# LIS-TU-Berlin/SVN-ICP

Hardware: AMD Instinct MI355X
Metric: scan-pair registrations/sec at N particles x M source pts, 1/2/4/8 GPU (higher is better)
Workload: dtype f64; 1 GPU; C3: 128 particles SVN-ICP, 131072-pt source vs 262144-pt target, K=100, I=20, max_dist=1.0, lr=1.0, SVNFullGrad=False, correspondence=fast, early stop off; synthetic 64-beam scans (seed 20250718); particles=128, target_points=262144, knn_count=100, parallelism=single GPU

## Files before the change

include/svnicp_hip.h:

```cpp
#ifndef SVNICP_HIP_H
#define SVNICP_HIP_H

#include <stdint.h>

#ifdef __cplusplus
extern "C" {
#endif

#define SVNICP_ABI_VERSION 1

typedef struct svnicp_ctx svnicp_ctx;

#define SVNICP_ALIGN_SUCCESS 1
#define SVNICP_NO_OPTIMIZER 2

typedef enum {
  SVNICP_OK = 0,
  SVNICP_ERR_INVALID = -1,
  SVNICP_ERR_HIP = -2,
  SVNICP_ERR_NO_DEVICE = -3,
  SVNICP_ERR_NOMEM = -4
} svnicp_status;

#define SVNICP_MODE_SVN 0
#define SVNICP_MODE_SVGD 1

#define SVNICP_OPT_ADAM 0
#define SVNICP_OPT_RMSPROP 1
#define SVNICP_OPT_SGD 2
#define SVNICP_OPT_ADAGRAD 3
#define SVNICP_OPT_NONE (-1)

#define SVNICP_MEM_HOST 0
#define SVNICP_MEM_DEVICE 1

typedef struct svnicp_params {
  int32_t struct_size;
  int32_t mode;
  int32_t iterations;
  int32_t knn_count;
  double lr;
  double max_dist;
  double convergence_threshold;
  int32_t check_early_stop;
  int32_t svn_full_grad;
  int32_t optimizer;
  int32_t record_trace;
} svnicp_params;

int svnicp_create(const svnicp_params *params, int device, const double *init_pose6xP, int P,
                  svnicp_ctx **out);
void svnicp_destroy(svnicp_ctx *ctx);
const char *svnicp_last_error(const svnicp_ctx *ctx);
int svnicp_abi_version(void);

#define SVNICP_OWN_STREAM ((void *)(intptr_t)-1)
int svnicp_set_stream(svnicp_ctx *ctx, void *hip_stream);
int svnicp_synchronize(svnicp_ctx *ctx);

int svnicp_set_clouds(svnicp_ctx *ctx, const double *src_xyz, int64_t B, const double *tgt_xyz,
                      int64_t M, int mem_kind);
int svnicp_set_particles(svnicp_ctx *ctx, const double *init_pose6xP, int P);
int svnicp_set_source(svnicp_ctx *ctx, const double *src_xyz, int64_t B, int mem_kind);
int svnicp_set_target(svnicp_ctx *ctx, const double *tgt_xyz, int64_t M, int mem_kind);

int svnicp_set_initial_mean(svnicp_ctx *ctx, const double R0_rowmajor[9], const double t0[3]);
int svnicp_set_k(svnicp_ctx *ctx, int k);
int svnicp_set_max_dist(svnicp_ctx *ctx, double max_dist);

int svnicp_align(svnicp_ctx *ctx);
int svnicp_align_async(svnicp_ctx *ctx);

int svnicp_get_transformation(svnicp_ctx *ctx, double out6[6]);
int svnicp_get_distribution(svnicp_ctx *ctx, double out6[6]);
int svnicp_get_cov_matrix(svnicp_ctx *ctx, double out36[36]);
int svnicp_get_particles(svnicp_ctx *ctx, double *out6P);
int svnicp_get_particle_weight(svnicp_ctx *ctx, double *outP);
int svnicp_get_particle_history(svnicp_ctx *ctx, float *outIx6P);
int svnicp_get_runtime(svnicp_ctx *ctx, double out3[3]);

int svnicp_set_option(svnicp_ctx *ctx, const char *name, const char *value);

int svnicp_set_shard(svnicp_ctx *ctx, int p_lo, int p_hi);
int svnicp_set_row_shard(svnicp_ctx *ctx, int row_rank, int row_world, int64_t total_source_points);
void *svnicp_rank_sums_devptr(svnicp_ctx *ctx);
int svnicp_align_begin(svnicp_ctx *ctx);
int svnicp_stage_candidates(svnicp_ctx *ctx, int64_t b_lo, int64_t b_hi);
int svnicp_build_candidate_table(svnicp_ctx *ctx);
int svnicp_iter_accumulate(svnicp_ctx *ctx, int iteration);
int svnicp_iter_update(svnicp_ctx *ctx, int iteration);
int svnicp_finish(svnicp_ctx *ctx);
int svnicp_stopped(svnicp_ctx *ctx);
void *svnicp_candidates_devptr(svnicp_ctx *ctx);
void *svnicp_sums_devptr(svnicp_ctx *ctx);
#define SVNICP_NSUMS 22

typedef struct svnicp_map svnicp_map;
int svnicp_map_create(int device, double voxel_size, double max_range, int max_points, int64_t capacity_voxels,
                      svnicp_map **out);
void svnicp_map_destroy(svnicp_map *map);
const char *svnicp_map_last_error(const svnicp_map *map);
int svnicp_map_clear(svnicp_map *map);
int svnicp_map_size(svnicp_map *map, int64_t *voxels);
int svnicp_map_add_cloud(svnicp_map *map, const float *xyz, int64_t n, int mem_kind, const double R_rowmajor[9],
                         const double t[3]);
int svnicp_map_skipped_points(svnicp_map *map, int64_t *out);
int svnicp_map_query(svnicp_map *map, const double center[3], double max_range, int64_t *count_out);
void *svnicp_map_points_devptr(svnicp_map *map);
int svnicp_map_download(svnicp_map *map, double *out_xyz, int64_t cap_points, int64_t *n_out);

int svnicp_get_candidates(svnicp_ctx *ctx, int32_t *outBK);
int svnicp_get_candidate_dist2(svnicp_ctx *ctx, double *outBK);
int svnicp_get_trace(svnicp_ctx *ctx, int32_t *corr, double *H, double *b, double *newton,
                     double *phi, double *h);
int svnicp_get_iterations_run(svnicp_ctx *ctx, int *out);
int svnicp_get_gpu_ms(svnicp_ctx *ctx, double out3[3]);

int svnicp_get_knn_fallbacks(svnicp_ctx *ctx, int *out);
int svnicp_get_knn_fallback_rows(svnicp_ctx *ctx, int32_t *out, int cap, int *n_out);
int svnicp_get_knn_survivors(svnicp_ctx *ctx, int32_t *outB);
int svnicp_get_ambiguous_steps(svnicp_ctx *ctx, int *out);
int svnicp_get_ambiguous_pairs(svnicp_ctx *ctx, int64_t *out);
#define SVNICP_KERNEL_CLASSES 6
int svnicp_set_profile(svnicp_ctx *ctx, int on);
int svnicp_get_kernel_ms(svnicp_ctx *ctx, double *ms6, int32_t *launches6);

typedef struct svnicp_prep svnicp_prep;
int svnicp_prep_create(int device, svnicp_prep **out);
void svnicp_prep_destroy(svnicp_prep *prep);
const char *svnicp_prep_last_error(const svnicp_prep *prep);
int svnicp_prep_scan(svnicp_prep *prep, const float *xyz, int64_t n, int mem_kind, double min_range, double max_range,
                     double voxel_size, double *scan_max_range, int64_t *n_cropped, int64_t *n_map, int64_t *n_source);
const float *svnicp_prep_cropped_devptr(svnicp_prep *prep);
const float *svnicp_prep_map_cloud_devptr(svnicp_prep *prep);
const double *svnicp_prep_source_devptr(svnicp_prep *prep);
const float *svnicp_prep_source_f32_devptr(svnicp_prep *prep);
int svnicp_prep_download(svnicp_prep *prep, int which , float *out_xyz,
                         int64_t cap_points, int64_t *n_out);

#define SVNICP_STAMP_F64 0
#define SVNICP_STAMP_F32 1
#define SVNICP_STAMP_U32 2
#define SVNICP_DESKEW_KITTI 1
int svnicp_prep_scan_deskew(svnicp_prep *prep, const float *xyz, const void *stamps, int stamp_type, int64_t n, int mem_kind,
                            const double delta_xi[6], int flags, double min_range, double max_range, double voxel_size,
                            double *scan_max_range, int64_t *n_cropped, int64_t *n_map, int64_t *n_source);
const float *svnicp_prep_deskewed_devptr(svnicp_prep *prep);
int svnicp_prep_download_deskewed(svnicp_prep *prep, float *out_xyz, int64_t cap_points, int64_t *n_out);

typedef struct svnicp_seg_params {
  int32_t struct_size;
  int32_t n_scan, horizon_scan, ground_scan_ind;
  float ang_res_x, ang_res_y, ang_bottom;
  float min_range, mount_angle, segment_theta;
  int32_t valid_point_num, valid_line_num;
} svnicp_seg_params;
#define SVNICP_SEG_VLP16 0
#define SVNICP_SEG_HDL32E 1
#define SVNICP_SEG_HDL64E 2
#define SVNICP_SEG_VLS128 3
#define SVNICP_SEG_RS32 4
#define SVNICP_SEG_OS1_16 5
#define SVNICP_SEG_OS1_64 6
#define SVNICP_SEG_OS0_128 7
int svnicp_seg_default_params(int sensor, svnicp_seg_params *out);
int svnicp_prep_segment(svnicp_prep *prep, const float *xyz, int64_t n, int mem_kind, const svnicp_seg_params *params,
                        int64_t *n_segmented);
const float *svnicp_prep_segmented_devptr(svnicp_prep *prep);
const int32_t *svnicp_prep_segmented_index_devptr(svnicp_prep *prep);
int svnicp_prep_download_segmented(svnicp_prep *prep, float *out_xyz, int32_t *out_index, int64_t cap_points, int64_t *n_out);
int svnicp_prep_download_seg_images(svnicp_prep *prep, int32_t *owner, float *range, int8_t *ground, int32_t *label,
                                    int64_t cap_pixels);

#ifdef __cplusplus
}
#endif
#endif
```

svn-icp_amd/binding.py:

```python
from __future__ import annotations

import ctypes as C
import os
import re

_HERE = os.path.dirname(os.path.abspath(__file__))
_ROOT = os.path.dirname(_HERE)
_LIB_PATH = os.path.join(_HERE, "libsvnicp_hip.so")
_HEADER = os.path.join(_ROOT, "include", "svnicp_hip.h")


class SvnIcpError(RuntimeError):
    pass


class Params(C.Structure):
    _fields_ = [("struct_size", C.c_int32), ("mode", C.c_int32), ("iterations", C.c_int32),
                ("knn_count", C.c_int32), ("lr", C.c_double), ("max_dist", C.c_double),
                ("convergence_threshold", C.c_double), ("check_early_stop", C.c_int32),
                ("svn_full_grad", C.c_int32), ("optimizer", C.c_int32), ("record_trace", C.c_int32)]


class SegParamsStruct(C.Structure):
    _fields_ = [("struct_size", C.c_int32), ("n_scan", C.c_int32), ("horizon_scan", C.c_int32), ("ground_scan_ind", C.c_int32),
                ("ang_res_x", C.c_float), ("ang_res_y", C.c_float), ("ang_bottom", C.c_float), ("min_range", C.c_float),
                ("mount_angle", C.c_float), ("segment_theta", C.c_float), ("valid_point_num", C.c_int32),
                ("valid_line_num", C.c_int32)]


def library_path() -> str:
    return _LIB_PATH


def declared_symbols() -> list[str]:
    txt = open(_HEADER).read()
    txt = re.sub(r"/\*.*?\*/", "", txt, flags=re.S)
    return sorted(set(re.findall(r"\b(svnicp_[a-z0-9_]+)\s*\(", txt)))


_lib = None


def load_library():
    global _lib
    if _lib is not None:
        return _lib
    if not os.path.exists(_LIB_PATH):
        raise SvnIcpError(f"{_LIB_PATH} is missing: build it with `python -c 'import __graft_entry__ as g; g.build()'` "
                          "(hipcc --offload-arch=gfx950). There is no CPU fallback.")
    try:
        import torch
    except ImportError:
        pass
    try:
        L = C.CDLL(_LIB_PATH)
    except OSError as e:
        raise SvnIcpError(f"cannot load {_LIB_PATH}: {e}") from e
    dp, fp, ip = C.POINTER(C.c_double), C.POINTER(C.c_float), C.POINTER(C.c_int32)
    vp = C.c_void_p
    L.svnicp_abi_version.restype = C.c_int
    L.svnicp_last_error.restype = C.c_char_p
    L.svnicp_last_error.argtypes = [vp]
    L.svnicp_create.argtypes = [C.POINTER(Params), C.c_int, dp, C.c_int, C.POINTER(vp)]
    L.svnicp_destroy.argtypes = [vp]
    L.svnicp_destroy.restype = None
    L.svnicp_set_stream.argtypes = [vp, vp]
    L.svnicp_synchronize.argtypes = [vp]
    L.svnicp_set_clouds.argtypes = [vp, vp, C.c_int64, vp, C.c_int64, C.c_int]
    L.svnicp_set_particles.argtypes = [vp, dp, C.c_int]
    L.svnicp_set_source.argtypes = [vp, vp, C.c_int64, C.c_int]
    L.svnicp_set_target.argtypes = [vp, vp, C.c_int64, C.c_int]
    L.svnicp_map_create.argtypes = [C.c_int, C.c_double, C.c_double, C.c_int, C.c_int64, C.POINTER(vp)]
    L.svnicp_map_destroy.argtypes = [vp]
    L.svnicp_map_destroy.restype = None
    L.svnicp_map_last_error.argtypes = [vp]
    L.svnicp_map_last_error.restype = C.c_char_p
    L.svnicp_map_clear.argtypes = [vp]
    L.svnicp_map_size.argtypes = [vp, C.POINTER(C.c_int64)]
    L.svnicp_map_add_cloud.argtypes = [vp, vp, C.c_int64, C.c_int, dp, dp]
    L.svnicp_map_query.argtypes = [vp, dp, C.c_double, C.POINTER(C.c_int64)]
    L.svnicp_map_points_devptr.argtypes = [vp]
    L.svnicp_map_points_devptr.restype = vp
    L.svnicp_map_download.argtypes = [vp, dp, C.c_int64, C.POINTER(C.c_int64)]
    L.svnicp_prep_create.argtypes = [C.c_int, C.POINTER(vp)]
    L.svnicp_prep_destroy.argtypes = [vp]
    L.svnicp_prep_destroy.restype = None
    L.svnicp_prep_last_error.argtypes = [vp]
    L.svnicp_prep_last_error.restype = C.c_char_p
    L.svnicp_prep_scan.argtypes = [vp, vp, C.c_int64, C.c_int, C.c_double, C.c_double, C.c_double, dp, C.POINTER(C.c_int64),
                                   C.POINTER(C.c_int64), C.POINTER(C.c_int64)]
    L.svnicp_map_skipped_points.argtypes = [vp, C.POINTER(C.c_int64)]
    for name in ("svnicp_prep_cropped_devptr", "svnicp_prep_map_cloud_devptr", "svnicp_prep_source_devptr", "svnicp_prep_source_f32_devptr"):
        getattr(L, name).argtypes = [vp]
        getattr(L, name).restype = vp
    L.svnicp_prep_download.argtypes = [vp, C.c_int, vp, C.c_int64, C.POINTER(C.c_int64)]
    L.svnicp_prep_scan_deskew.argtypes = [vp, vp, vp, C.c_int, C.c_int64, C.c_int, dp, C.c_int, C.c_double, C.c_double, C.c_double, dp,
                                          C.POINTER(C.c_int64), C.POINTER(C.c_int64), C.POINTER(C.c_int64)]
    L.svnicp_prep_deskewed_devptr.argtypes = [vp]
    L.svnicp_prep_deskewed_devptr.restype = vp
    L.svnicp_prep_download_deskewed.argtypes = [vp, vp, C.c_int64, C.POINTER(C.c_int64)]
    L.svnicp_seg_default_params.argtypes = [C.c_int, C.POINTER(SegParamsStruct)]
    L.svnicp_prep_segment.argtypes = [vp, vp, C.c_int64, C.c_int, C.POINTER(SegParamsStruct), C.POINTER(C.c_int64)]
    for name in ("svnicp_prep_segmented_devptr", "svnicp_prep_segmented_index_devptr"):
        getattr(L, name).argtypes = [vp]
        getattr(L, name).restype = vp
    L.svnicp_prep_download_segmented.argtypes = [vp, vp, vp, C.c_int64, C.POINTER(C.c_int64)]
    L.svnicp_prep_download_seg_images.argtypes = [vp, vp, vp, vp, vp, C.c_int64]
    L.svnicp_set_initial_mean.argtypes = [vp, dp, dp]
    L.svnicp_set_k.argtypes = [vp, C.c_int]
    L.svnicp_set_option.argtypes = [vp, C.c_char_p, C.c_char_p]
    L.svnicp_set_max_dist.argtypes = [vp, C.c_double]
    L.svnicp_align.argtypes = [vp]
    L.svnicp_align_async.argtypes = [vp]
    for n in ("transformation", "distribution", "cov_matrix", "particles", "particle_weight", "runtime",
              "candidate_dist2", "gpu_ms"):
        getattr(L, "svnicp_get_" + n).argtypes = [vp, dp]
    L.svnicp_get_particle_history.argtypes = [vp, fp]
    L.svnicp_get_candidates.argtypes = [vp, ip]
    L.svnicp_get_trace.argtypes = [vp, ip, dp, dp, dp, dp, dp]
    L.svnicp_get_knn_fallbacks.argtypes = [vp, C.POINTER(C.c_int)]
    L.svnicp_get_knn_survivors.argtypes = [vp, ip]
    L.svnicp_get_knn_fallback_rows.argtypes = [vp, ip, C.c_int, C.POINTER(C.c_int)]
    L.svnicp_get_ambiguous_steps.argtypes = [vp, C.POINTER(C.c_int)]
    L.svnicp_get_ambiguous_pairs.argtypes = [vp, C.POINTER(C.c_int64)]
    L.svnicp_get_iterations_run.argtypes = [vp, C.POINTER(C.c_int)]
    L.svnicp_set_profile.argtypes = [vp, C.c_int]
    L.svnicp_get_kernel_ms.argtypes = [vp, dp, ip]
    L.svnicp_set_shard.argtypes = [vp, C.c_int, C.c_int]
    L.svnicp_set_row_shard.argtypes = [vp, C.c_int, C.c_int, C.c_int64]
    L.svnicp_rank_sums_devptr.argtypes = [vp]
    L.svnicp_rank_sums_devptr.restype = vp
    L.svnicp_align_begin.argtypes = [vp]
    L.svnicp_stage_candidates.argtypes = [vp, C.c_int64, C.c_int64]
    L.svnicp_build_candidate_table.argtypes = [vp]
    L.svnicp_iter_accumulate.argtypes = [vp, C.c_int]
    L.svnicp_iter_update.argtypes = [vp, C.c_int]
    L.svnicp_finish.argtypes = [vp]
    L.svnicp_stopped.argtypes = [vp]
    L.svnicp_candidates_devptr.argtypes = [vp]
    L.svnicp_candidates_devptr.restype = vp
    L.svnicp_sums_devptr.argtypes = [vp]
    L.svnicp_sums_devptr.restype = vp
    for name in declared_symbols():
        getattr(L, name)
    _lib = L
    return L


def abi_version() -> int:
    return int(load_library().svnicp_abi_version())
```

svn-icp_amd/csrc/api.hip:

```cpp
#include "../../include/svnicp_hip.h"

#include <cmath>
#include <algorithm>
#include <cstdio>
#include <cstdlib>
#include <cstring>
#include <string>
#include <vector>

#include "kernels.hpp"

using namespace svnicp;

namespace {

thread_local std::string g_create_error;

template <typename T>
struct DevBuf {
  T* p = nullptr;
  size_t cap = 0;
  hipError_t ensure(size_t n) {
    if (n <= cap && p) return hipSuccess;
    if (p) { (void)hipFree(p); p = nullptr; cap = 0; }
    if (n == 0) n = 1;
    hipError_t e = hipMalloc(reinterpret_cast<void**>(&p), n * sizeof(T));
    if (e == hipSuccess) cap = n;
    return e;
  }
  void release() { if (p) (void)hipFree(p); p = nullptr; cap = 0; }
};

}

struct svnicp_ctx {
  svnicp_params prm{};
  int device = 0;
  int num_cus = 256;
  hipStream_t own_stream = nullptr, stream = nullptr;
  hipStream_t side = nullptr;
  hipEvent_t ev_fork = nullptr, ev_join = nullptr, ev_init = nullptr;
  hipEvent_t ev_chunk[3] = {nullptr, nullptr, nullptr};
  int* h_flags = nullptr;
  bool init_in_flight = false;
  bool median_pending = false;
  double* h_init = nullptr; size_t h_init_cap = 0;
  double* h_stats = nullptr; size_t h_stats_cap = 0;
  bool host_stats_valid = false;
  int single_done_it = -1;
  hipEvent_t ev[3] = {nullptr, nullptr, nullptr};
  std::string err;

  int64_t B = 0, M = 0, Mp = 0;
  int K = 0, S = 0, P = 0;
  int p_lo = 0, p_hi = 0;
  bool src_set = false, tgt_set = false;
  bool clouds_set = false, particles_set = false, particles_dirty = false, shard_set = false;
  bool began = false, have_candidates = false, have_result = false;
  Pose0 pose0{};
  AccumPlan plan{};
  int plan_P = -1; int64_t plan_B = -1; int plan_K = -1;

  DevBuf<double> eul, opt, uctl;
  DevBuf<double> src, tgt, tx, ty, tz, pool_d, cand_d2, table, init_pose, R, t, Rtot, pose_out, sums, partial, work,
      stats, trH, trb, trN, trphi, trh;
  DevBuf<int32_t> pool_i, cand_idx, trcorr, torig, pool2, fail_list;
  DevBuf<float> txf, tyf, tzf, cmaxb;
  DevBuf<float4> tablef, tablea;
  DevBuf<unsigned int> small_bar;
  bool small_launched = false;
  bool defer_fin = false;
  DevBuf<uint8_t> kbest;
  DevBuf<int32_t> kidx;
  int row_rank = 0, row_world = 1;
  int64_t B_total = 0;
  DevBuf<double> rank_sums;
  DevBuf<double> sl_d, fail_tau, anchor, qrec;
  DevBuf<int32_t> sl_i;
  int sliced_max = 0;
  DevBuf<int> ambig;
  int accum_mode = 3;
  DevBuf<unsigned long long> emax;
  DevBuf<int> fail_count;
  DevBuf<int> stage_fail_count;
  DevBuf<int32_t> stage_fail_list;
  int knn_variant = 0;
  int target_layout = -1;
  DevBuf<unsigned int> keys_a, keys_b;
  DevBuf<int32_t> vals_a, order_t, qorder, stat_n;
  DevBuf<unsigned long long> bbox;
  DevBuf<float> tile_box;
  DevBuf<unsigned char> sort_tmp;
  size_t sort_tmp_bytes = 0;
  bool use_scan = false;
  int64_t scan_Ms = 0; int scan_rank = 0, scan_S2 = 0;
  DevBuf<float> history;
  DevBuf<int> ctl;
  int hist_I = 0, hist_P = 0;
  Tuning tune{};
  DevBuf<double> full_q, full_d2;
  DevBuf<int32_t> arena, chunk_tab;
  int arena_cap = 0;
  DevBuf<int32_t> full_idx;
  unsigned long long* dbg_phase = nullptr;
  unsigned long long* dbg_upd = nullptr;
  bool finish_seen = true;
  int finish_iter = 0;
  double gpu_ms[3] = {0, 0, 0};
  bool timing_valid = false;
  bool profile = false;
  unsigned profile_mask = 0;
  int pcur = -1;
  std::vector<hipEvent_t> pev;
  std::vector<int> pcls;
  size_t pused = 0;
};

constexpr int kFallbackGrid = 256;
constexpr int kFallbackSlicedMax = 512;
constexpr int kFallbackQW = 2;

enum { KC_KNN = 0, KC_TABLE = 1, KC_SEARCH = 2, KC_ACCUM = 3, KC_REDUCE = 4, KC_UPDATE = 5, KC_COUNT = SVNICP_KERNEL_CLASSES };

static hipError_t prof_begin(svnicp_ctx* c, int cls) {
  c->pcur = -1;
  if (!c->profile || !((c->profile_mask >> cls) & 1u)) return hipSuccess;
  c->pcur = cls;
  if (c->pused * 2 + 2 > c->pev.size()) {
    for (int i = 0; i < 2; ++i) {
      hipEvent_t e;
      hipError_t r = hipEventCreate(&e);
      if (r != hipSuccess) return r;
      c->pev.push_back(e);
    }
    c->pcls.push_back(cls);
  }
  c->pcls[c->pused] = cls;
  return hipEventRecord(c->pev[2 * c->pused], c->stream);
}
static hipError_t prof_end(svnicp_ctx* c) {
  if (!c->profile || c->pcur < 0) return hipSuccess;
  c->pcur = -1;
  hipError_t r = hipEventRecord(c->pev[2 * c->pused + 1], c->stream);
  c->pused += 1;
  return r;
}

#define CTX_CHECK(ctx)                         \
  do {                                         \
    if (!(ctx)) return SVNICP_ERR_INVALID;     \
  } while (0)

static int fail(svnicp_ctx* c, int code, const std::string& msg) {
  if (c) c->err = msg; else g_create_error = msg;
  return code;
}
#define HIPCHK(c, expr)                                                                          \
  do {                                                                                           \
    hipError_t _e = (expr);                                                                      \
    if (_e != hipSuccess)                                                                        \
      return fail((c), _e == hipErrorOutOfMemory ? SVNICP_ERR_NOMEM : SVNICP_ERR_HIP,           \
                  std::string(#expr) + ": " + hipGetErrorString(_e));                            \
  } while (0)

static int bind(svnicp_ctx* c) {
  HIPCHK(c, hipSetDevice(c->device));
  return 0;
}

extern "C" {

int svnicp_abi_version(void) { return SVNICP_ABI_VERSION; }

const char* svnicp_last_error(const svnicp_ctx* ctx) { return ctx ? ctx->err.c_str() : g_create_error.c_str(); }

int svnicp_create(const svnicp_params* params, int device, const double* init_pose6xP, int P, svnicp_ctx** out) {
  if (!params || !out) return fail(nullptr, SVNICP_ERR_INVALID, "svnicp_create: null argument");
  if (params->struct_size != (int32_t)sizeof(svnicp_params))
    return fail(nullptr, SVNICP_ERR_INVALID, "svnicp_create: svnicp_params.struct_size mismatch");
  if (params->iterations < 0 || params->knn_count < 1)
    return fail(nullptr, SVNICP_ERR_INVALID, "svnicp_create: iterations >= 0 and knn_count >= 1 required");
  if (params->mode != SVNICP_MODE_SVN && params->mode != SVNICP_MODE_SVGD)
    return fail(nullptr, SVNICP_ERR_INVALID, "svnicp_create: unknown mode");
  int ndev = 0;
  if (hipGetDeviceCount(&ndev) != hipSuccess || ndev <= 0)
    return fail(nullptr, SVNICP_ERR_NO_DEVICE, "svnicp_create: no HIP device visible (this library has no CPU path)");
  if (device < 0 || device >= ndev) return fail(nullptr, SVNICP_ERR_INVALID, "svnicp_create: bad device ordinal");
  hipDeviceProp_t prop;
  if (hipSetDevice(device) != hipSuccess || hipGetDeviceProperties(&prop, device) != hipSuccess)
    return fail(nullptr, SVNICP_ERR_HIP, "svnicp_create: hipGetDeviceProperties failed");
  if (std::strncmp(prop.gcnArchName, "gfx950", 6) != 0)
    return fail(nullptr, SVNICP_ERR_NO_DEVICE,
                std::string("svnicp_create: device is ") + prop.gcnArchName + ", this library carries gfx950 code only");
  svnicp_ctx* c = new svnicp_ctx();
  c->prm = *params;
  c->device = device;
  c->num_cus = prop.multiProcessorCount > 0 ? prop.multiProcessorCount : 256;
  c->K = params->knn_count;
  c->finish_iter = params->iterations;
  const double I3[9] = {1, 0, 0, 0, 1, 0, 0, 0, 1};
  std::memcpy(c->pose0.R0, I3, sizeof I3);
  c->pose0.t0[0] = c->pose0.t0[1] = c->pose0.t0[2] = 0.0;
  if (hipStreamCreateWithFlags(&c->own_stream, hipStreamNonBlocking) != hipSuccess) {
    delete c;
    return fail(nullptr, SVNICP_ERR_HIP, "svnicp_create: hipStreamCreate failed");
  }
  c->stream = c->own_stream;
  if (hipStreamCreateWithFlags(&c->side, hipStreamNonBlocking) != hipSuccess ||
      hipEventCreateWithFlags(&c->ev_fork, hipEventDisableTiming) != hipSuccess ||
      hipEventCreateWithFlags(&c->ev_join, hipEventDisableTiming) != hipSuccess ||
      hipEventCreateWithFlags(&c->ev_init, hipEventDisableTiming) != hipSuccess) {
    svnicp_destroy(c);
    return fail(nullptr, SVNICP_ERR_HIP, "svnicp_create: hipStreamCreate / hipEventCreate failed");
  }
  for (auto& e : c->ev)
    if (hipEventCreate(&e) != hipSuccess) { delete c; return fail(nullptr, SVNICP_ERR_HIP, "hipEventCreate failed"); }
  if (c->ctl.ensure(4) != hipSuccess) { delete c; return fail(nullptr, SVNICP_ERR_NOMEM, "hipMalloc failed"); }
  *out = c;
  if (const char* e = getenv("SVNICP_OPTIONS")) {
    std::string all(e);
    size_t pos = 0;
    while (pos < all.size()) {
      const size_t end = all.find(';', pos) == std::string::npos ? all.size() : all.find(';', pos);
      const std::string kv = all.substr(pos, end - pos);
      const size_t eq = kv.find('=');
      if (eq != std::string::npos && svnicp_set_option(c, kv.substr(0, eq).c_str(), kv.substr(eq + 1).c_str()) != 0) {
        g_create_error = c->err; svnicp_destroy(c); *out = nullptr; return SVNICP_ERR_INVALID;
      }
      pos = end + 1;
    }
  }
  if (init_pose6xP) {
    int rc = svnicp_set_particles(c, init_pose6xP, P);
    if (rc != 0) { g_create_error = c->err; svnicp_destroy(c); *out = nullptr; return rc; }
  }
  return SVNICP_OK;
}

void svnicp_destroy(svnicp_ctx* c) {
  if (!c) return;
  (void)hipSetDevice(c->device);
  if (c->stream) (void)hipStreamSynchronize(c->stream);
  if (c->side) { (void)hipStreamSynchronize(c->side); (void)hipStreamDestroy(c->side); }
  if (c->h_init) (void)hipHostFree(c->h_init);
  if (c->h_stats) (void)hipHostFree(c->h_stats);
  if (c->ev_fork) (void)hipEventDestroy(c->ev_fork);
  if (c->ev_join) (void)hipEventDestroy(c->ev_join);
  if (c->ev_init) (void)hipEventDestroy(c->ev_init);
  for (auto& e : c->ev_chunk) if (e) (void)hipEventDestroy(e);
  if (c->h_flags) (void)hipHostFree(c->h_flags);
  DevBuf<double>* dbl[] = {&c->src, &c->tgt, &c->tx, &c->ty, &c->tz, &c->pool_d, &c->cand_d2, &c->table,
                           &c->init_pose, &c->R, &c->t, &c->Rtot, &c->pose_out, &c->sums, &c->partial, &c->work,
                           &c->stats, &c->trH, &c->trb, &c->trN, &c->trphi, &c->trh};
  for (auto* b : dbl) b->release();
  c->eul.release(); c->opt.release(); c->uctl.release(); c->rank_sums.release(); c->stage_fail_count.release(); c->stage_fail_list.release(); c->small_bar.release();
  c->keys_a.release(); c->keys_b.release(); c->vals_a.release(); c->order_t.release(); c->qorder.release(); c->stat_n.release(); c->bbox.release(); c->tile_box.release(); c->sort_tmp.release();
  c->full_q.release(); c->full_d2.release(); c->full_idx.release(); c->arena.release(); c->chunk_tab.release();
  c->pool_i.release(); c->torig.release(); c->pool2.release(); c->fail_list.release(); c->txf.release(); c->tyf.release(); c->tzf.release(); c->cmaxb.release(); c->tablef.release(); c->tablea.release(); c->kbest.release(); c->kidx.release(); c->sl_d.release(); c->sl_i.release(); c->fail_tau.release(); c->qrec.release(); c->anchor.release(); c->ambig.release(); c->emax.release(); c->fail_count.release(); c->cand_idx.release(); c->trcorr.release(); c->history.release(); c->ctl.release();
  if (c->dbg_phase) (void)hipFree(c->dbg_phase);
  if (c->dbg_upd) (void)hipFree(c->dbg_upd);
  for (auto& e : c->ev) if (e) (void)hipEventDestroy(e);
  for (auto& e : c->pev) (void)hipEventDestroy(e);
  if (c->own_stream) (void)hipStreamDestroy(c->own_stream);
  delete c;
}

int svnicp_set_stream(svnicp_ctx* c, void* hip_stream) {
  CTX_CHECK(c);
  if (bind(c)) return SVNICP_ERR_HIP;
  HIPCHK(c, hipStreamSynchronize(c->stream));
  c->stream = hip_stream == SVNICP_OWN_STREAM ? c->own_stream : reinterpret_cast<hipStream_t>(hip_stream);
  return SVNICP_OK;
}

static int check_small_kernel(svnicp_ctx* c);
int svnicp_synchronize(svnicp_ctx* c) {
  CTX_CHECK(c);
  if (bind(c)) return SVNICP_ERR_HIP;
  HIPCHK(c, hipStreamSynchronize(c->stream));
  if (const int rc = check_small_kernel(c)) return rc;
  if (c->have_result && c->h_stats) c->host_stats_valid = true;
  return SVNICP_OK;
}

int svnicp_set_source(svnicp_ctx* c, const double* src, int64_t B, int mem_kind) {
  CTX_CHECK(c);
  if (!src || B < 1) return fail(c, SVNICP_ERR_INVALID, "svnicp_set_source: need B >= 1");
  if (B > 0x7fffffffLL) return fail(c, SVNICP_ERR_INVALID, "svnicp_set_source: cloud too large");
  if (bind(c)) return SVNICP_ERR_HIP;
  HIPCHK(c, c->src.ensure((size_t)B * 3));
  const hipMemcpyKind kind = mem_kind == SVNICP_MEM_DEVICE ? hipMemcpyDeviceToDevice : hipMemcpyHostToDevice;
  HIPCHK(c, hipMemcpyAsync(c->src.p, src, (size_t)B * 24, kind, c->stream));
  if (mem_kind != SVNICP_MEM_DEVICE) HIPCHK(c, hipStreamSynchronize(c->stream));
  c->B = B;
  c->src_set = true;
  c->clouds_set = c->src_set && c->tgt_set;
  c->have_candidates = false;
  return SVNICP_OK;
}

int svnicp_set_target(svnicp_ctx* c, const double* tgt, int64_t M, int mem_kind) {
  CTX_CHECK(c);
  if (!tgt || M < 1) return fail(c, SVNICP_ERR_INVALID, "svnicp_set_target: need M >= 1");
  if (M > 0x7fffffffLL) return fail(c, SVNICP_ERR_INVALID, "svnicp_set_target: cloud too large");
  if (bind(c)) return SVNICP_ERR_HIP;
  HIPCHK(c, c->tgt.ensure((size_t)M * 3));
  const hipMemcpyKind kind = mem_kind == SVNICP_MEM_DEVICE ? hipMemcpyDeviceToDevice : hipMemcpyHostToDevice;
  HIPCHK(c, hipMemcpyAsync(c->tgt.p, tgt, (size_t)M * 24, kind, c->stream));
  if (mem_kind != SVNICP_MEM_DEVICE) HIPCHK(c, hipStreamSynchronize(c->stream));
  c->M = M; c->Mp = knn_padded_targets(M);
  c->target_layout = -1;
  c->tgt_set = true;
  c->clouds_set = c->src_set && c->tgt_set;
  c->have_candidates = false;
  return SVNICP_OK;
}

int svnicp_set_clouds(svnicp_ctx* c, const double* src, int64_t B, const double* tgt, int64_t M, int mem_kind) {
  CTX_CHECK(c);
  if (!src || !tgt || B < 1 || M < 1) return fail(c, SVNICP_ERR_INVALID, "svnicp_set_clouds: need B >= 1, M >= 1");
  if (M > 0x7fffffffLL || B > 0x7fffffffLL) return fail(c, SVNICP_ERR_INVALID, "svnicp_set_clouds: cloud too large");
  int rc = svnicp_set_source(c, src, B, mem_kind);
  if (rc) return rc;
  return svnicp_set_target(c, tgt, M, mem_kind);
}

int svnicp_set_particles(svnicp_ctx* c, const double* init, int P) {
  CTX_CHECK(c);
  if (!init || P < 1) return fail(c, SVNICP_ERR_INVALID, "svnicp_set_particles: need P >= 1");
  if (bind(c)) return SVNICP_ERR_HIP;
  HIPCHK(c, c->init_pose.ensure((size_t)P * 6));
  HIPCHK(c, c->R.ensure((size_t)P * 9));
  HIPCHK(c, c->t.ensure((size_t)P * 3));
  HIPCHK(c, c->Rtot.ensure((size_t)P * 12));
  HIPCHK(c, c->pose_out.ensure((size_t)P * 6));
  HIPCHK(c, c->sums.ensure((size_t)P * kNSums));
  HIPCHK(c, c->stats.ensure((size_t)48 + P));
  HIPCHK(c, c->work.ensure(update_workspace_doubles(P)));
  HIPCHK(c, c->eul.ensure((size_t)P * 6));
  HIPCHK(c, c->opt.ensure((size_t)P * 18));
  HIPCHK(c, c->uctl.ensure(update_uctl_doubles(P)));
  if ((size_t)P * 6 > c->h_init_cap || (size_t)P + 48 > c->h_stats_cap) {
    HIPCHK(c, hipStreamSynchronize(c->stream));
    if (c->h_init) (void)hipHostFree(c->h_init);
    if (c->h_stats) (void)hipHostFree(c->h_stats);
    c->h_init = c->h_stats = nullptr; c->h_init_cap = c->h_stats_cap = 0;
    HIPCHK(c, hipHostMalloc(reinterpret_cast<void**>(&c->h_init), (size_t)P * 48, hipHostMallocDefault));
    HIPCHK(c, hipHostMalloc(reinterpret_cast<void**>(&c->h_stats), ((size_t)P + 48) * 8, hipHostMallocDefault));
    c->h_init_cap = (size_t)P * 6; c->h_stats_cap = (size_t)P + 48;
  } else if (c->init_in_flight) {
    HIPCHK(c, hipEventSynchronize(c->ev_init));
  }
  std::memcpy(c->h_init, init, (size_t)P * 48);
  HIPCHK(c, hipMemcpyAsync(c->init_pose.p, c->h_init, (size_t)P * 48, hipMemcpyHostToDevice, c->stream));
  HIPCHK(c, hipEventRecord(c->ev_init, c->stream));
  c->init_in_flight = true;
  c->host_stats_valid = false;
  const bool first = !c->particles_set || P != c->P;
  if (first && c->row_world > 1) { c->row_world = 1; c->row_rank = 0; c->B_total = 0; }
  c->P = P;
  if (!c->shard_set || first) { c->p_lo = 0; c->p_hi = P; c->shard_set = false; }
  HIPCHK(c, launch_init_particles(c->init_pose.p, P, c->pose0, c->prm.mode, c->R.p, c->t.p, c->Rtot.p, c->pose_out.p,
                                  (first || c->prm.mode == SVNICP_MODE_SVN) ? 1 : 0, c->eul.p, c->stream));
  c->particles_set = true;
  c->particles_dirty = true;
  return SVNICP_OK;
}

int svnicp_set_initial_mean(svnicp_ctx* c, const double R0[9], const double t0[3]) {
  CTX_CHECK(c);
  if (!R0 || !t0) return fail(c, SVNICP_ERR_INVALID, "svnicp_set_initial_mean: null argument");
  std::memcpy(c->pose0.R0, R0, 9 * sizeof(double));
  std::memcpy(c->pose0.t0, t0, 3 * sizeof(double));
  c->have_candidates = false;
  return SVNICP_OK;
}

int svnicp_set_k(svnicp_ctx* c, int k) {
  CTX_CHECK(c);
  if (k < 1) return fail(c, SVNICP_ERR_INVALID, "svnicp_set_k: k >= 1 required");
  c->K = k;
  c->have_candidates = false;
  return SVNICP_OK;
}

int svnicp_set_max_dist(svnicp_ctx* c, double md) {
  CTX_CHECK(c);
  c->prm.max_dist = md;
  return SVNICP_OK;
}

int svnicp_set_option(svnicp_ctx* c, const char* name, const char* value) {
  CTX_CHECK(c);
  if (!name || !value) return fail(c, SVNICP_ERR_INVALID, "svnicp_set_option: null argument");
  const std::string k(name), v(value);
  Tuning& t = c->tune;
  auto num = [&](int lo, int hi, int* out) { char* end = nullptr; const long x = strtol(v.c_str(), &end, 10);
                                             if (end == v.c_str() || *end || x < lo || x > hi) return false; *out = (int)x; return true; };
  bool ok = true;
  if (k == "knn") { if (v == "auto") t.knn = -1; else if (v == "v1") t.knn = 0; else if (v == "v2") t.knn = 1; else if (v == "brute") t.knn = 2; else if (v == "tiles") t.knn = 3; else ok = false; }
  else if (k == "fallback_sliced_max") ok = num(-1, 1 << 20, &t.fallback_sliced_max);
  else if (k == "accum") { if (v == "f64") t.accum = 0; else if (v == "valu") t.accum = 1; else if (v == "split") t.accum = 3; else ok = false; }
  else if (k == "update") { if (v == "auto") t.update_fused = 0; else if (v == "fused") t.update_fused = 1; else ok = false; }
  else if (k == "fused_update_max_p") ok = num(1, 700, &t.fused_update_max_p);
  else if (k == "wgpcu") { int x = 0, y = 0; ok = sscanf(v.c_str(), "%d,%d", &x, &y) == 2 && x >= 0 && x <= 64 && y >= 0 && y <= 16; if (ok) { t.wgpcu_search = x; t.wgpcu_accum = y; } }
  else if (k == "tp") ok = num(0, 1 << 16, &t.tp);
  else if (k == "debug") ok = num(0, 1, &t.debug);
  else if (k == "scan_split") ok = num(0, 16, &t.scan_split);
  else if (k == "group_stride") ok = num(0, 1 << 30, &t.group_stride);
  else if (k == "accum_min_steps") ok = num(0, 1 << 20, &t.accum_min_steps);
  else if (k == "brute_qb") { ok = num(0, 6, &t.brute_qb); }
  else if (k == "single") { if (v == "fused") t.single_fused = 1; else if (v == "split") t.single_fused = 0; else ok = false; }
  else if (k == "chain") { if (v == "auto") { t.small_chain = 1; t.persistent = 0; } else if (v == "persistent") { t.small_chain = 1; t.persistent = 1; }
                           else if (v == "general") { t.small_chain = 0; t.persistent = 0; } else ok = false; }
  else if (k == "median") { if (v == "auto") t.median_inline = -1; else if (v == "stream") t.median_inline = 0; else if (v == "inline") t.median_inline = 1; else ok = false; }
  else if (k == "correspondence") { if (v == "fast") t.full_corr = 0; else if (v == "full") t.full_corr = 1; else ok = false; }
  else return fail(c, SVNICP_ERR_INVALID, "svnicp_set_option: unknown option '" + k + "'");
  if (!ok) return fail(c, SVNICP_ERR_INVALID, "svnicp_set_option: bad value '" + v + "' for option '" + k + "'");
  c->have_candidates = false;
  c->target_layout = -1;
  return SVNICP_OK;
}

int svnicp_set_shard(svnicp_ctx* c, int p_lo, int p_hi) {
  CTX_CHECK(c);
  if (!c->particles_set || p_lo < 0 || p_hi > c->P || p_lo > p_hi)
    return fail(c, SVNICP_ERR_INVALID, "svnicp_set_shard: need 0 <= p_lo <= p_hi <= P after svnicp_set_particles");
  c->p_lo = p_lo; c->p_hi = p_hi; c->shard_set = true;
  return SVNICP_OK;
}

int svnicp_set_row_shard(svnicp_ctx* c, int row_rank, int row_world, int64_t total_source_points) {
  CTX_CHECK(c);
  if (!c->particles_set || row_world < 1 || row_rank < 0 || row_rank >= row_world || (row_world > 1 && total_source_points < 1))
    return fail(c, SVNICP_ERR_INVALID, "svnicp_set_row_shard: need 0 <= row_rank < row_world and the whole scan's point count, after svnicp_set_particles");
  if (bind(c)) return SVNICP_ERR_HIP;
  c->row_rank = row_rank; c->row_world = row_world;
  c->B_total = row_world > 1 ? total_source_points : 0;
  if (row_world > 1) {
    HIPCHK(c, c->rank_sums.ensure((size_t)row_world * c->P * kNSums));
    HIPCHK(c, hipMemsetAsync(c->rank_sums.p, 0, (size_t)row_world * c->P * kNSums * sizeof(double), c->stream));
  }
  return SVNICP_OK;
}

void* svnicp_rank_sums_devptr(svnicp_ctx* c) { return (c && c->row_world > 1) ? (void*)c->rank_sums.p : nullptr; }

static int ensure_target_layout(svnicp_ctx* c) {
  int want = 0;
  if (knn_tiles_applicable(c->Mp, c->K)) want = 2;
  else if (knn_scan_plan(c->Mp, c->K, &c->scan_Ms, &c->scan_rank, &c->scan_S2)) want = 1;
  if (c->tune.knn == 0) want = 0;
  if (c->tune.knn == 1) want = knn_scan_plan(c->Mp, c->K, &c->scan_Ms, &c->scan_rank, &c->scan_S2) ? 1 : 0;
  if ((c->tune.knn == -1 && knn_brute_applicable(c->B, c->M, c->K)) || (c->tune.knn == 2 && c->K <= 128 && c->M < (1ll << 31))) want = 3;
  c->knn_variant = want;
  c->use_scan = want == 1;
  if (want == 3) return 0;
  const int layout = want == 2 ? 1 : 0;
  if (c->target_layout == layout) return 0;
  const int64_t M = c->M, Mp = c->Mp;
  HIPCHK(c, c->tx.ensure((size_t)Mp)); HIPCHK(c, c->ty.ensure((size_t)Mp)); HIPCHK(c, c->tz.ensure((size_t)Mp));
  HIPCHK(c, c->txf.ensure((size_t)Mp)); HIPCHK(c, c->tyf.ensure((size_t)Mp)); HIPCHK(c, c->tzf.ensure((size_t)Mp));
  HIPCHK(c, c->torig.ensure((size_t)Mp));
  HIPCHK(c, c->emax.ensure(1));
  if (layout == 0) {
    HIPCHK(c, launch_targets_soa2(c->tgt.p, M, Mp, c->tx.p, c->ty.p, c->tz.p, c->txf.p, c->tyf.p, c->tzf.p, c->torig.p,
                                  c->emax.p, c->stream));
  } else {
    const size_t nmax = (size_t)(M > c->B ? M : c->B);
    HIPCHK(c, c->keys_a.ensure(nmax)); HIPCHK(c, c->keys_b.ensure(nmax)); HIPCHK(c, c->vals_a.ensure(nmax));
    HIPCHK(c, c->order_t.ensure((size_t)M)); HIPCHK(c, c->qorder.ensure((size_t)c->B));
    HIPCHK(c, c->bbox.ensure(6));
    HIPCHK(c, c->tile_box.ensure((size_t)6 * (Mp / 512)));
    const size_t tb = sort_temp_bytes(nmax);
    if (tb > c->sort_tmp_bytes) { HIPCHK(c, c->sort_tmp.ensure(tb)); c->sort_tmp_bytes = tb; }
    HIPCHK(c, launch_bbox(c->tgt.p, M, c->bbox.p, c->stream));
    HIPCHK(c, launch_morton_order(c->tgt.p, 0, M, 0, c->pose0, c->bbox.p, c->keys_a.p, c->keys_b.p, c->vals_a.p,
                                  c->order_t.p, c->sort_tmp.p, c->sort_tmp_bytes, c->stream));
    HIPCHK(c, launch_targets_sorted(c->tgt.p, M, Mp, c->order_t.p, c->tx.p, c->ty.p, c->tz.p, c->txf.p, c->tyf.p, c->tzf.p,
                                    c->torig.p, c->tile_box.p, c->emax.p, c->stream));
  }
  c->target_layout = layout;
  return 0;
}

int svnicp_align_begin(svnicp_ctx* c) {
  CTX_CHECK(c);
  if (!c->clouds_set || !c->particles_set)
    return fail(c, SVNICP_ERR_INVALID, "svnicp_align: svnicp_set_clouds and svnicp_set_particles must come first");
  if (bind(c)) return SVNICP_ERR_HIP;
  const int I = c->prm.iterations, P = c->P;
  const int64_t B = c->B;
  c->S = knn_pool_size(c->K);
  HIPCHK(c, hipEventRecord(c->ev[0], c->stream));
  if (ensure_target_layout(c)) return c->err.empty() ? SVNICP_ERR_HIP : SVNICP_ERR_HIP;
  if (c->knn_variant == 3) {
    HIPCHK(c, c->fail_count.ensure(1));
  } else if (c->knn_variant != 0) {
    if (c->knn_variant == 2) {
      c->scan_S2 = kTilesBase + kTilesChunks * kTilesChunk;
      c->arena_cap = (int)std::max<int64_t>(32768, B / 4);
      HIPCHK(c, c->pool2.ensure((size_t)B * kTilesBase));
      HIPCHK(c, c->arena.ensure((size_t)c->arena_cap * kTilesChunk));
      HIPCHK(c, c->chunk_tab.ensure((size_t)B * kTilesChunks + 16 + (size_t)(B + 63) / 64 + 1));
    } else {
      HIPCHK(c, c->pool2.ensure((size_t)B * c->scan_S2));
    }
    HIPCHK(c, c->fail_list.ensure((size_t)B));
    HIPCHK(c, c->fail_count.ensure(1));
    HIPCHK(c, c->fail_tau.ensure((size_t)B));
    HIPCHK(c, c->qrec.ensure((size_t)B * 6));
    HIPCHK(c, c->pool_d.ensure((size_t)kFallbackGrid * 4 * kFallbackQW * c->S));
    HIPCHK(c, c->pool_i.ensure((size_t)kFallbackGrid * 4 * kFallbackQW * c->S));
    c->sliced_max = c->tune.fallback_sliced_max >= 0 ? c->tune.fallback_sliced_max : kFallbackSlicedMax;
    if (c->sliced_max > kFallbackSlicedMax) c->sliced_max = kFallbackSlicedMax;
    if (c->sliced_max > 0) {
      HIPCHK(c, c->sl_d.ensure((size_t)c->sliced_max * knn_slice_count(c->K) * c->K));
      HIPCHK(c, c->sl_i.ensure((size_t)c->sliced_max * knn_slice_count(c->K) * c->K));
    }
  } else {
    HIPCHK(c, c->pool_d.ensure((size_t)B * c->S));
    HIPCHK(c, c->pool_i.ensure((size_t)B * c->S));
  }
  HIPCHK(c, c->cand_idx.ensure((size_t)B * c->K));
  HIPCHK(c, c->cand_d2.ensure((size_t)B * c->K));
  c->accum_mode = c->tune.accum;
  HIPCHK(c, c->cmaxb.ensure((size_t)B));
  HIPCHK(c, c->ambig.ensure(2));
  HIPCHK(c, c->history.ensure((size_t)(I > 0 ? I : 1) * 6 * P));
  c->hist_I = I; c->hist_P = P;
  const int nshard = c->p_hi - c->p_lo;
  if (nshard > 0) {
    Tuning tn = c->tune;
    tn.small_chain = tn.small_chain && P >= 2 && P <= 128 && P <= tn.fused_update_max_p && !tn.update_fused && c->row_world == 1 &&
                     c->p_lo == 0 && c->p_hi == P && !tn.full_corr;
    c->plan = plan_accumulate(nshard, B, c->K, c->num_cus, c->accum_mode, tn);
    if (c->tune.debug)
      fprintf(stderr, "[svnicp] stage-B plan: mode=%d PW=%d WP=%d TP=%d grid=%dx%d tiles/block=%d smem=%zu sgrid=%d pts/block=%d/%d\n", c->plan.f32,
              c->plan.PW, c->plan.WP, c->plan.TP, c->plan.grid_x, c->plan.grid_y, c->plan.tiles_per_block, c->plan.smem,
              c->plan.sgrid_x, c->plan.spts_per_block, c->plan.pts_per_block);
    if (c->plan.smem > 160u * 1024)
      return fail(c, SVNICP_ERR_INVALID, "svnicp_align: knn_count " + std::to_string(c->K) + " needs " + std::to_string(c->plan.smem) +
                  " bytes of LDS per workgroup (limit 163840): the candidate count is too large for this particle count");
    HIPCHK(c, c->partial.ensure((size_t)std::max(c->plan.grid_x, P == 1 ? single_particle_grid(B) : 0) * c->plan.Ppad * kNSums));
  } else {
    c->plan = AccumPlan{};
    c->plan.f32 = c->accum_mode == 3 ? 1 : c->accum_mode;
  }
  if (c->plan.f32 != 3) HIPCHK(c, c->table.ensure((size_t)B * c->K * 3));
  if (c->plan.f32 == 3) { HIPCHK(c, c->tablea.ensure((size_t)B * 128)); HIPCHK(c, c->anchor.ensure((size_t)B * 3)); }
  if (c->plan.f32 == 3) { HIPCHK(c, c->kbest.ensure((size_t)B * c->plan.Ppad)); HIPCHK(c, c->kidx.ensure((size_t)B * c->plan.Ppad)); }
  else HIPCHK(c, c->tablef.ensure((size_t)B * c->K));
  if (c->prm.record_trace) {
    HIPCHK(c, c->trcorr.ensure((size_t)I * P * B));
    HIPCHK(c, c->trH.ensure((size_t)I * P * 36));
    HIPCHK(c, c->trb.ensure((size_t)I * P * 6));
    HIPCHK(c, c->trN.ensure((size_t)I * P * 6));
    HIPCHK(c, c->trphi.ensure((size_t)I * P * 6));
    HIPCHK(c, c->trh.ensure((size_t)I + 1));
    HIPCHK(c, hipMemsetAsync(c->trcorr.p, 0xff, (size_t)I * P * B * 4, c->stream));
    HIPCHK(c, hipMemsetAsync(c->trH.p, 0, (size_t)I * P * 36 * 8, c->stream));
    HIPCHK(c, hipMemsetAsync(c->trb.p, 0, (size_t)I * P * 6 * 8, c->stream));
    HIPCHK(c, hipMemsetAsync(c->trN.p, 0, (size_t)I * P * 6 * 8, c->stream));
    HIPCHK(c, hipMemsetAsync(c->trphi.p, 0, (size_t)I * P * 6 * 8, c->stream));
    HIPCHK(c, hipMemsetAsync(c->trh.p, 0, ((size_t)I + 1) * 8, c->stream));
  }
  c->pused = 0;
  c->single_done_it = -1;
  if (c->median_pending) HIPCHK(c, hipStreamWaitEvent(c->stream, c->ev_join, 0));
  c->median_pending = false;
  if (!c->finish_seen && c->prm.mode == SVNICP_MODE_SVGD && c->prm.check_early_stop) {
    int v[2] = {0, 0};
    HIPCHK(c, hipMemcpyAsync(v, c->ctl.p, sizeof v, hipMemcpyDeviceToHost, c->stream));
    HIPCHK(c, hipStreamSynchronize(c->stream));
    if (v[0]) c->finish_iter = v[1];
    c->finish_seen = true;
  }
  {
    BeginZero z{};
    auto add = [&](void* p, size_t bytes) { if (p && bytes) { z.ptr[z.n] = static_cast<unsigned int*>(p); z.dwords[z.n] = (unsigned int)(bytes / 4); ++z.n; } };
    add(c->uctl.p, update_uctl_doubles(P) * sizeof(double));
    add(c->history.p, (size_t)(I > 0 ? I : 1) * 6 * P * sizeof(float));
    add(c->ambig.p, 2 * sizeof(int));
    if (c->knn_variant == 3) add(c->fail_count.p, sizeof(int));
    HIPCHK(c, c->small_bar.ensure(8));
    add(c->small_bar.p, 8 * sizeof(unsigned int));
    if (c->prm.mode == SVNICP_MODE_SVGD) add(c->opt.p, (size_t)P * 18 * sizeof(double));
    z.ctl = c->ctl.p; z.iterations = I;
    HIPCHK(c, launch_init_particles(c->init_pose.p, P, c->pose0, 2, c->R.p, c->t.p, c->Rtot.p, c->pose_out.p, 0,
                                    nullptr, c->stream, &z));
  }
  c->particles_dirty = false;
  c->began = true;
  c->finish_seen = false;
  c->have_result = false;
  c->timing_valid = false;
  return SVNICP_OK;
}

static hipError_t launch_fallback(svnicp_ctx* c, KnnArgs a) {
  a.qlist = c->fail_list.p; a.qlist_count = c->fail_count.p; a.list_grid = kFallbackGrid; a.list_qw = kFallbackQW;
  a.slice_max_queries = c->sliced_max; a.slices = 0;
  hipError_t e = launch_knn_topk(a, c->stream);
  if (e != hipSuccess || c->sliced_max <= 0) return e;
  a.slices = knn_slice_count(a.K);
  a.merge_n = 1;
  while (a.merge_n < a.slices * a.K) a.merge_n <<= 1;
  a.sl_d = c->sl_d.p; a.sl_i = c->sl_i.p;
  e = launch_knn_topk(a, c->stream);
  if (e != hipSuccess) return e;
  return launch_knn_merge_slices(a, c->stream);
}

static int stage_a(svnicp_ctx* c, const double* qsrc, const Pose0& pose, int K, int32_t* out_idx, double* out_d2, int64_t b_lo,
                   int64_t b_hi) {
  KnnArgs a{};
  a.src = qsrc; a.pose = pose; a.tx = c->tx.p; a.ty = c->ty.p; a.tz = c->tz.p; a.torig = c->torig.p;
  a.M = c->M; a.Mp = c->Mp; a.b_lo = b_lo; a.b_hi = b_hi; a.K = K; a.S = knn_pool_size(K);
  a.pool_d = c->pool_d.p; a.pool_i = c->pool_i.p; a.out_idx = out_idx; a.out_d2 = out_d2;
  if (c->knn_variant == 3) {
    KnnBruteArgs k{};
    k.src = qsrc; k.pose = pose; k.tgt = c->tgt.p; k.M = c->M; k.b_lo = b_lo; k.b_hi = b_hi; k.K = K; k.out_idx = out_idx; k.out_d2 = out_d2;
    if (c->tune.debug) {
      if (!c->dbg_phase) HIPCHK(c, hipMalloc(&c->dbg_phase, (8 + 8 * 65536) * sizeof(unsigned long long)));
      HIPCHK(c, hipMemsetAsync(c->dbg_phase, 0, 8 * sizeof(unsigned long long), c->stream));
      k.phase_cycles = c->dbg_phase;
    }
    HIPCHK(c, launch_knn_brute(k, c->num_cus, c->tune.brute_qb, c->stream));
    if (k.phase_cycles) {
      unsigned long long h[8];
      HIPCHK(c, hipMemcpyAsync(h, c->dbg_phase, sizeof h, hipMemcpyDeviceToHost, c->stream));
      HIPCHK(c, hipStreamSynchronize(c->stream));
      const int qb = c->tune.brute_qb > 0 ? c->tune.brute_qb : knn_brute_queries_per_block(b_hi - b_lo, c->num_cus);
      const double nwg = (double)((b_hi - b_lo + qb - 1) / qb);
      fprintf(stderr, "[svnicp] k_knn_brute (%d queries per workgroup) thread-0 cycles per workgroup: pass A %.0f, bound %.0f, pass B %.0f, general path %.0f, rank + write %.0f\n",
              qb, h[0] / nwg, h[1] / nwg, h[2] / nwg, h[3] / nwg, h[4] / nwg);
    }
  } else if (c->knn_variant == 2) {
    const int64_t n = b_hi - b_lo;
    if (n > 0) {
      HIPCHK(c, launch_morton_order(qsrc, b_lo, n, 1, pose, c->bbox.p, c->keys_a.p, c->keys_b.p, c->vals_a.p,
                                    c->qorder.p + b_lo, c->sort_tmp.p, c->sort_tmp_bytes, c->stream));
      KnnTilesArgs k{};
      k.src = qsrc; k.pose = pose; k.qorder = c->qorder.p + b_lo;
      k.tx = c->tx.p; k.ty = c->ty.p; k.tz = c->tz.p; k.txf = c->txf.p; k.tyf = c->tyf.p; k.tzf = c->tzf.p;
      k.torig = c->torig.p; k.tile_box = c->tile_box.p; k.emax_bits = c->emax.p;
      k.M = c->M; k.Mp = c->Mp; k.n_tiles = (int)(c->Mp / 512); k.b_lo = b_lo; k.b_hi = b_hi; k.K = K; k.S2 = c->scan_S2;
      k.pool = c->pool2.p; k.out_idx = out_idx; k.out_d2 = out_d2;
      k.arena = c->arena.p; k.chunk_tab = c->chunk_tab.p; k.arena_cap = c->arena_cap; k.tab_rows = c->B;
      k.scan_split = c->tune.scan_split == 4 ? 4 : 8;
      {
        const unsigned int ng = (unsigned int)((n + 63) / 64);
        unsigned int st = c->tune.group_stride > 0 ? (unsigned int)c->tune.group_stride : 17u;
        auto gcd = [](unsigned int x, unsigned int y) { while (y) { const unsigned int t = x % y; x = y; y = t; } return x; };
        while (st > 1 && gcd(st, ng) != 1) st += 2;
        if (ng <= 2 || st >= ng) st = 1;
        k.group_stride = st;
      }
      HIPCHK(c, hipMemsetAsync(c->chunk_tab.p, 0xff, ((size_t)c->B * kTilesChunks + 16 + (size_t)(c->B + 63) / 64 + 1) * sizeof(int32_t), c->stream));
      k.fail_list = c->fail_list.p; k.fail_count = c->fail_count.p; k.fail_tau = c->fail_tau.p; k.qrec = c->qrec.p;
      a.qthr = c->fail_tau.p;
      if (c->prm.record_trace) { HIPCHK(c, c->stat_n.ensure((size_t)c->B)); k.stat_n = c->stat_n.p; }
      HIPCHK(c, hipMemsetAsync(c->fail_count.p, 0, sizeof(int), c->stream));
      unsigned long long*& dbg_phase = c->dbg_phase;
      const size_t dbg_waves = (size_t)((n + 63) / 64) * 4;
      if (c->tune.debug && dbg_waves <= 65536) {
        if (!dbg_phase) HIPCHK(c, hipMalloc(&dbg_phase, (8 + 8 * 65536) * sizeof(unsigned long long)));
        HIPCHK(c, hipMemsetAsync(dbg_phase, 0, (8 + 8 * dbg_waves) * sizeof(unsigned long long), c->stream));
        k.phase_cycles = dbg_phase;
      }
      HIPCHK(c, launch_knn_tiles(k, c->stream));
      if (k.phase_cycles) {
        std::vector<unsigned long long> h(8 + 8 * dbg_waves);
        HIPCHK(c, hipMemcpyAsync(h.data(), dbg_phase, h.size() * sizeof(unsigned long long), hipMemcpyDeviceToHost, c->stream));
        HIPCHK(c, hipStreamSynchronize(c->stream));
        fprintf(stderr, "[svnicp] k_knn_tiles wave cycles: rank %llu seed %llu scan %llu barrier waits + hand-over %llu | counts: seed tiles %llu scan tiles %llu scan (query, tile) pairs %llu\n", h[0], h[1], h[2], h[3], h[4], h[5], h[6]);
        auto column = [&](const char* tag, int col, unsigned long long floor_) {
          std::vector<unsigned long long> v;
          for (size_t w = 0; w < dbg_waves; ++w) { const unsigned long long x = h[8 + 8 * w + col]; if (x >= floor_) v.push_back(x); }
          if (v.empty()) return;
          std::sort(v.begin(), v.end());
          fprintf(stderr, "[svnicp]   seed kernel %-12s n %6zu  p50 %8llu  p90 %8llu  p99 %8llu  max %8llu cycles\n", tag, v.size(), v[v.size() / 2],
                  v[v.size() * 9 / 10], v[v.size() * 99 / 100], v.back());
        };
        column("rank", 0, 5000); column("seed", 1, 1); column("tile loop", 5, 1); column("bisection", 6, 1); column("waits", 3, 0);
      }
      HIPCHK(c, launch_fallback(c, a));
    }
  } else if (c->use_scan && K == c->K) {
    KnnScanArgs k{};
    k.src = qsrc; k.pose = pose; k.tx = c->tx.p; k.ty = c->ty.p; k.tz = c->tz.p;
    k.txf = c->txf.p; k.tyf = c->tyf.p; k.tzf = c->tzf.p; k.torig = c->torig.p; k.emax_bits = c->emax.p;
    k.M = c->M; k.Mp = c->Mp; k.Ms = c->scan_Ms; k.b_lo = b_lo; k.b_hi = b_hi; k.K = K; k.S2 = c->scan_S2;
    k.seed_rank = c->scan_rank; k.pool = c->pool2.p; k.out_idx = out_idx; k.out_d2 = out_d2;
    k.fail_list = c->fail_list.p; k.fail_count = c->fail_count.p;
    HIPCHK(c, hipMemsetAsync(c->fail_count.p, 0, sizeof(int), c->stream));
    HIPCHK(c, launch_knn_scan(k, c->stream));
    HIPCHK(c, launch_fallback(c, a));
  } else {
    if (c->knn_variant != 0) return fail(c, SVNICP_ERR_INVALID, "correspondence = full needs knn_count <= 128 (Morton-tile stage A) or knn = v1");
    HIPCHK(c, launch_knn_topk(a, c->stream));
  }
  return SVNICP_OK;
}

int svnicp_stage_candidates(svnicp_ctx* c, int64_t b_lo, int64_t b_hi) {
  CTX_CHECK(c);
  if (!c->began) return fail(c, SVNICP_ERR_INVALID, "svnicp_stage_candidates: call svnicp_align_begin first");
  if (b_lo < 0 || b_hi > c->B || b_lo > b_hi) return fail(c, SVNICP_ERR_INVALID, "svnicp_stage_candidates: bad row range");
  if (bind(c)) return SVNICP_ERR_HIP;
  HIPCHK(c, prof_begin(c, KC_KNN));
  const int rc = stage_a(c, c->src.p, c->pose0, c->K, c->cand_idx.p, c->cand_d2.p, b_lo, b_hi);
  if (rc) return rc;
  if (c->tune.full_corr && c->knn_variant != 0 && c->knn_variant != 3) {
    HIPCHK(c, c->stage_fail_count.ensure(1)); HIPCHK(c, c->stage_fail_list.ensure((size_t)c->B));
    HIPCHK(c, hipMemcpyAsync(c->stage_fail_count.p, c->fail_count.p, sizeof(int), hipMemcpyDeviceToDevice, c->stream));
    HIPCHK(c, hipMemcpyAsync(c->stage_fail_list.p, c->fail_list.p, (size_t)c->B * sizeof(int32_t), hipMemcpyDeviceToDevice, c->stream));
  }
  HIPCHK(c, prof_end(c));
  return SVNICP_OK;
}


int svnicp_build_candidate_table(svnicp_ctx* c) {
  CTX_CHECK(c);
  if (!c->began) return fail(c, SVNICP_ERR_INVALID, "svnicp_build_candidate_table: call svnicp_align_begin first");
  if (bind(c)) return SVNICP_ERR_HIP;
  HIPCHK(c, prof_begin(c, KC_TABLE));
  if (c->plan.f32 == 3)
    HIPCHK(c, launch_build_table3(c->cand_idx.p, c->B, c->K, c->tgt.p, c->M, c->plan.f32 == 3 ? nullptr : c->table.p,
                                  c->anchor.p, c->tablea.p, c->cmaxb.p, c->stream));
  else
    HIPCHK(c, launch_build_table2(c->cand_idx.p, c->B, c->K, c->tgt.p, c->M, c->table.p, c->tablef.p, c->cmaxb.p, c->stream));
  HIPCHK(c, prof_end(c));
  HIPCHK(c, hipEventRecord(c->ev[1], c->stream));
  c->have_candidates = true;
  return SVNICP_OK;
}

static UpdateArgs update_args(svnicp_ctx* c, int it) {
  UpdateArgs u{};
  u.sums = c->row_world > 1 ? c->rank_sums.p : c->sums.p; u.n_ranks = c->row_world; u.R = c->R.p; u.t = c->t.p; u.Rtot = c->Rtot.p; u.pose = c->pose0;
  u.P = c->P; u.iteration = it; u.iterations = c->prm.iterations;
  u.lr = c->prm.lr; u.conv_thr = c->prm.convergence_threshold;
  u.check_early_stop = c->prm.check_early_stop; u.full_grad = c->prm.svn_full_grad;
  u.work = c->work.p; u.history = c->history.p; u.pose_out = c->pose_out.p; u.ctl = c->ctl.p;
  if (c->prm.record_trace) {
    u.trH = c->trH.p + (size_t)it * c->P * 36; u.trb = c->trb.p + (size_t)it * c->P * 6;
    u.trN = c->trN.p + (size_t)it * c->P * 6; u.trphi = c->trphi.p + (size_t)it * c->P * 6; u.trh = c->trh.p + it;
  }
  u.eul = c->eul.p; u.opt = c->opt.p; u.optimizer = c->prm.optimizer;
  u.n_src = (double)(c->row_world > 1 ? c->B_total : c->B);
  u.uctl = c->uctl.p;
  u.dbg = c->tune.debug ? c->dbg_upd : nullptr;
  u.svgd = c->prm.mode == SVNICP_MODE_SVGD ? 1 : 0;
  return u;
}
static bool update_one_kernel(const svnicp_ctx* c) { return c->P < 2 || (c->tune.update_fused && c->P <= c->tune.fused_update_max_p); }

static bool small_chain(const svnicp_ctx* c) { return c->plan.f32 == 3 && c->plan.small && c->plan.grid_x <= kSmallChainBlocks; }

constexpr int kMedianInlineMaxP = 128;
static bool median_inline(const svnicp_ctx* c) {
  if (c->P < 2 || c->P > 128 || c->P > c->tune.fused_update_max_p || update_one_kernel(c)) return false;
  return c->tune.median_inline == 1 || (c->tune.median_inline == -1 && c->P <= kMedianInlineMaxP);
}

static int fork_median(svnicp_ctx* c, int it) {
  if (update_one_kernel(c) || c->median_pending || small_chain(c) || median_inline(c)) return SVNICP_OK;
  if (c->tune.debug && !c->dbg_upd) { HIPCHK(c, hipMalloc(&c->dbg_upd, 8 * sizeof(unsigned long long))); HIPCHK(c, hipMemset(c->dbg_upd, 0, 8 * sizeof(unsigned long long))); }
  const UpdateArgs u = update_args(c, it);
  HIPCHK(c, hipEventRecord(c->ev_fork, c->stream));
  HIPCHK(c, hipStreamWaitEvent(c->side, c->ev_fork, 0));
  HIPCHK(c, launch_update_median(u, c->num_cus, c->tune.fused_update_max_p, c->side));
  HIPCHK(c, hipEventRecord(c->ev_join, c->side));
  c->median_pending = true;
  return SVNICP_OK;
}

int svnicp_iter_accumulate(svnicp_ctx* c, int it) {
  CTX_CHECK(c);
  if (!c->began || !c->have_candidates)
    return fail(c, SVNICP_ERR_INVALID, "svnicp_iter_accumulate: candidates not staged");
  if (it < 0 || it >= c->prm.iterations) return fail(c, SVNICP_ERR_INVALID, "svnicp_iter_accumulate: bad iteration");
  if (bind(c)) return SVNICP_ERR_HIP;
  if (const int rc = fork_median(c, it)) return rc;
  const int nshard = c->p_hi - c->p_lo;
  if (nshard <= 0) return SVNICP_OK;
  AccumArgs a{};
  a.src = c->src.p; a.table = c->table.p; a.tablef = c->tablef.p; a.tablea = c->tablea.p; a.kbest = c->kbest.p; a.kidx = c->kidx.p; a.tgt = c->tgt.p; a.cand = c->cand_idx.p; a.anchor = c->anchor.p; a.M = c->M; a.cmax = c->cmaxb.p; a.ambig_count = c->ambig.p;
  a.Rtot = c->Rtot.p; a.B = c->B; a.K = c->K;
  a.p_lo = c->p_lo; a.p_hi = c->p_hi; a.max_dist = c->prm.max_dist; a.partial = c->partial.p; a.ctl = c->ctl.p;
  a.corr = c->prm.record_trace ? c->trcorr.p + (size_t)it * c->P * c->B : nullptr;
  a.svgd = c->prm.mode == SVNICP_MODE_SVGD ? 1 : 0;
  a.fin_iteration = -1;
  if (c->defer_fin && it >= 1) {
    const UpdateArgs up = update_args(c, it - 1);
    a.fin_iteration = it - 1; a.fin_P = c->P; a.fin_thr = c->prm.convergence_threshold; a.fin_norms = update_step_norms(up);
    a.fin_pose = c->pose_out.p; a.fin_history = c->history.p; a.fin_ctl = c->ctl.p;
  }
  if (c->tune.full_corr) {
    if (c->plan.f32 != 3) return fail(c, SVNICP_ERR_INVALID, "correspondence = full needs the split stage B (accum = split, more than 8 particles or knn_count <= 128)");
    HIPCHK(c, c->full_q.ensure((size_t)c->B * 3)); HIPCHK(c, c->full_d2.ensure((size_t)c->B));
    HIPCHK(c, c->full_idx.ensure((size_t)c->P * c->B));
    Pose0 ident{};
    ident.R0[0] = ident.R0[4] = ident.R0[8] = 1.0;
    HIPCHK(c, prof_begin(c, KC_SEARCH));
    for (int p = c->p_lo; p < c->p_hi; ++p) {
      HIPCHK(c, launch_transform_cloud(c->src.p, c->B, c->Rtot.p + 12 * (size_t)p, c->full_q.p, c->ctl.p, c->stream));
      const int rc = stage_a(c, c->full_q.p, ident, 1, c->full_idx.p + (size_t)p * c->B, c->full_d2.p, 0, c->B);
      if (rc) return rc;
    }
    HIPCHK(c, prof_end(c));
    a.full_idx = c->full_idx.p;
  } else if (c->plan.f32 == 3) {
    HIPCHK(c, prof_begin(c, KC_SEARCH));
    HIPCHK(c, launch_search_split(c->plan, a, c->stream));
    HIPCHK(c, prof_end(c));
  }
  const bool single = c->P == 1 && c->prm.mode == SVNICP_MODE_SVN && c->row_world == 1 && c->p_lo == 0 && c->p_hi == 1 &&
                      !c->tune.full_corr && c->tune.single_fused && accumulate_can_fuse_single(c->plan);
  const UpdateArgs us = update_args(c, it);
  a.ticket = reinterpret_cast<unsigned int*>(c->uctl.p + 41);
  HIPCHK(c, prof_begin(c, KC_ACCUM));
  HIPCHK(c, launch_accumulate(c->plan, a, single ? &us : nullptr, c->stream));
  HIPCHK(c, prof_end(c));
  if (single) { c->single_done_it = it; return SVNICP_OK; }
  if (small_chain(c)) return SVNICP_OK;
  HIPCHK(c, prof_begin(c, KC_REDUCE));
  double* rec = c->row_world > 1 ? c->rank_sums.p + (size_t)c->row_rank * c->P * kNSums : c->sums.p;
  HIPCHK(c, launch_reduce_partials(c->partial.p, c->plan.grid_x, c->plan.Ppad, c->p_lo, nshard, rec, c->ctl.p, c->stream));
  HIPCHK(c, prof_end(c));
  return SVNICP_OK;
}

int svnicp_iter_update(svnicp_ctx* c, int it) {
  CTX_CHECK(c);
  if (!c->began) return fail(c, SVNICP_ERR_INVALID, "svnicp_iter_update: call svnicp_align_begin first");
  if (it < 0 || it >= c->prm.iterations) return fail(c, SVNICP_ERR_INVALID, "svnicp_iter_update: bad iteration");
  if (bind(c)) return SVNICP_ERR_HIP;
  if (c->single_done_it == it) { c->single_done_it = -1; return SVNICP_OK; }
  if (c->tune.debug && !c->dbg_upd) { HIPCHK(c, hipMalloc(&c->dbg_upd, 8 * sizeof(unsigned long long))); HIPCHK(c, hipMemset(c->dbg_upd, 0, 8 * sizeof(unsigned long long))); }
  UpdateArgs u = update_args(c, it);
  HIPCHK(c, prof_begin(c, KC_UPDATE));
  if (c->tune.debug && it == c->prm.iterations - 1) {
    unsigned long long h[8];
    HIPCHK(c, hipStreamSynchronize(c->stream));
    HIPCHK(c, hipStreamSynchronize(c->side));
    HIPCHK(c, hipMemcpy(h, c->dbg_upd, sizeof(h), hipMemcpyDeviceToHost));
    fprintf(stderr, "[svnicp] Stein step thread-0 cycles (summed over launches so far; fused kernel: prepare / median / direction / pose / tail; k_upd_median: state / histogram / bin scan / collect / rank): %llu %llu %llu %llu %llu\n", h[0], h[1], h[2], h[3], h[4]);
  }
  if (update_one_kernel(c)) {
    u.svgd = 0;
    if (c->prm.mode == SVNICP_MODE_SVGD) HIPCHK(c, launch_update_svgd(u, c->stream));
    else HIPCHK(c, launch_update(u, c->stream));
  } else if (small_chain(c)) {
    u.sums = c->partial.p; u.n_ranks = c->plan.grid_x; u.sums_stride = c->plan.Ppad * kNSums; u.sums_out = c->sums.p;
    HIPCHK(c, launch_update_prepare_median(u, c->stream));
    HIPCHK(c, launch_update_direction(u, c->stream, !(c->defer_fin && it < c->prm.iterations - 1)));
  } else if (median_inline(c)) {
    HIPCHK(c, launch_update_prepare_median(u, c->stream));
    HIPCHK(c, launch_update_direction(u, c->stream, !(c->defer_fin && it < c->prm.iterations - 1)));
  } else {
    if (const int rc = fork_median(c, it)) return rc;
    HIPCHK(c, launch_update_prepare(u, c->stream));
    HIPCHK(c, hipStreamWaitEvent(c->stream, c->ev_join, 0));
    c->median_pending = false;
    HIPCHK(c, launch_update_direction(u, c->stream, !(c->defer_fin && it < c->prm.iterations - 1)));
  }
  HIPCHK(c, prof_end(c));
  return SVNICP_OK;
}

int svnicp_finish(svnicp_ctx* c) {
  CTX_CHECK(c);
  if (!c->began) return fail(c, SVNICP_ERR_INVALID, "svnicp_finish: call svnicp_align_begin first");
  if (bind(c)) return SVNICP_ERR_HIP;
  HIPCHK(c, hipEventRecord(c->ev[2], c->stream));
  StatsArgs s{c->pose_out.p, c->P, c->prm.mode, c->stats.p};
  HIPCHK(c, launch_stats(s, c->stream));
  c->host_stats_valid = false;
  if (c->h_stats && (size_t)c->P + 48 <= c->h_stats_cap)
    HIPCHK(c, hipMemcpyAsync(c->h_stats, c->stats.p, ((size_t)c->P + 48) * 8, hipMemcpyDeviceToHost, c->stream));
  c->have_result = true;
  c->timing_valid = true;
  return SVNICP_OK;
}

int svnicp_stopped(svnicp_ctx* c) {
  CTX_CHECK(c);
  if (bind(c)) return SVNICP_ERR_HIP;
  int v[2] = {0, 0};
  HIPCHK(c, hipMemcpyAsync(v, c->ctl.p, sizeof v, hipMemcpyDeviceToHost, c->stream));
  HIPCHK(c, hipStreamSynchronize(c->stream));
  return v[0] ? 1 : 0;
}

void* svnicp_candidates_devptr(svnicp_ctx* c) { return c ? (void*)c->cand_idx.p : nullptr; }
void* svnicp_sums_devptr(svnicp_ctx* c) { return c ? (void*)c->sums.p : nullptr; }

static int align_enqueue(svnicp_ctx* c, bool follow_stop) {
  CTX_CHECK(c);
  if (c->prm.mode == SVNICP_MODE_SVGD && (c->prm.optimizer < 0 || c->prm.optimizer > 3))
    return SVNICP_NO_OPTIMIZER;
  int rc = svnicp_align_begin(c);
  if (rc) return rc;
  if ((rc = svnicp_stage_candidates(c, 0, c->B))) return rc;
  if ((rc = svnicp_build_candidate_table(c))) return rc;
  c->small_launched = false;
  if (small_chain(c) && c->tune.persistent && !c->prm.record_trace && !c->profile && c->prm.iterations > 0 &&
      small_registration_supported(c->plan.PW, c->plan.WP, c->K)) {
    AccumArgs a{};
    a.src = c->src.p; a.tablea = c->tablea.p; a.kbest = c->kbest.p; a.kidx = c->kidx.p; a.tgt = c->tgt.p; a.cand = c->cand_idx.p;
    a.anchor = c->anchor.p; a.M = c->M; a.cmax = c->cmaxb.p; a.ambig_count = c->ambig.p;
    a.Rtot = c->Rtot.p; a.B = c->B; a.K = c->K; a.p_lo = c->p_lo; a.p_hi = c->p_hi; a.max_dist = c->prm.max_dist;
    a.partial = c->partial.p; a.ctl = c->ctl.p; a.svgd = c->prm.mode == SVNICP_MODE_SVGD ? 1 : 0;
    if (c->tune.debug && !c->dbg_upd) { HIPCHK(c, hipMalloc(&c->dbg_upd, 8 * sizeof(unsigned long long))); }
    if (c->tune.debug) HIPCHK(c, hipMemsetAsync(c->dbg_upd, 0, 8 * sizeof(unsigned long long), c->stream));
    UpdateArgs u = update_args(c, 0);
    u.sums_out = c->sums.p;
    const hipError_t e = launch_small_registration(c->plan, a, u, c->prm.iterations, c->small_bar.p, c->num_cus, c->stream);
    if (e == hipSuccess && c->tune.debug) {
      unsigned long long h[8];
      HIPCHK(c, hipStreamSynchronize(c->stream));
      HIPCHK(c, hipMemcpy(h, c->dbg_upd, sizeof h, hipMemcpyDeviceToHost));
      fprintf(stderr, "[svnicp] k_small_registration, workgroup 0, cycles over %d iterations: search %llu | barrier %llu | accumulate %llu | barrier %llu | prepare %llu | barrier %llu | direction %llu | barrier %llu\n",
              c->prm.iterations, h[0], h[1], h[2], h[3], h[4], h[5], h[6], h[7]);
    }
    if (e == hipSuccess) { c->small_launched = true; return svnicp_finish(c); }
    (void)hipGetLastError();
  }
  constexpr int kChunk = 4;
  const bool follow = follow_stop && c->prm.check_early_stop && c->prm.iterations > 2 * kChunk;
  if (follow && !c->h_flags) {
    HIPCHK(c, hipHostMalloc(reinterpret_cast<void**>(&c->h_flags), 3 * sizeof(int), hipHostMallocDefault));
    for (auto& e : c->ev_chunk) HIPCHK(c, hipEventCreateWithFlags(&e, hipEventDisableTiming));
  }
  c->defer_fin = c->prm.check_early_stop && !c->prm.record_trace && c->plan.f32 == 3 && !c->tune.full_corr && c->P >= 2 && !update_one_kernel(c);
  struct Reset { bool& f; ~Reset() { f = false; } } reset_defer{c->defer_fin};
  for (int it = 0; it < c->prm.iterations; ++it) {
    if ((rc = svnicp_iter_accumulate(c, it))) return rc;
    if ((rc = svnicp_iter_update(c, it))) return rc;
    if (follow && (it + 1) % kChunk == 0) {
      const int chunk = it / kChunk, slot = chunk % 3;
      HIPCHK(c, hipMemcpyAsync(&c->h_flags[slot], c->ctl.p, sizeof(int), hipMemcpyDeviceToHost, c->stream));
      HIPCHK(c, hipEventRecord(c->ev_chunk[slot], c->stream));
      if (chunk >= 1) {
        const int prev = (chunk - 1) % 3;
        HIPCHK(c, hipEventSynchronize(c->ev_chunk[prev]));
        if (c->h_flags[prev]) break;
      }
    }
  }
  return svnicp_finish(c);
}
int svnicp_align_async(svnicp_ctx* c) { return align_enqueue(c, false); }

static int check_small_kernel(svnicp_ctx* c) {
  if (!c->small_launched) return SVNICP_OK;
  c->small_launched = false;
  unsigned int w[2] = {0u, 0u};
  HIPCHK(c, hipMemcpyAsync(w, c->small_bar.p, sizeof w, hipMemcpyDeviceToHost, c->stream));
  HIPCHK(c, hipStreamSynchronize(c->stream));
  if (w[1] != 0u) { c->have_result = false; return fail(c, SVNICP_ERR_HIP, "svnicp_align: the small-registration kernel's grid barrier timed out (chain=persistent is an option; the default launches do not wait on each other)"); }
  return SVNICP_OK;
}

int svnicp_align(svnicp_ctx* c) {
  CTX_CHECK(c);
  if (c->shard_set && (c->p_lo != 0 || c->p_hi != c->P))
    return fail(c, SVNICP_ERR_INVALID, "svnicp_align: a particle shard is set; drive the split-phase calls instead");
  if (c->row_world > 1)
    return fail(c, SVNICP_ERR_INVALID, "svnicp_align: a source-row shard is set (this context holds a partial record); drive the split-phase calls instead");
  int rc = align_enqueue(c, true);
  if (rc) return rc;
  HIPCHK(c, hipStreamSynchronize(c->stream));
  if ((rc = check_small_kernel(c))) return rc;
  c->host_stats_valid = c->h_stats != nullptr;
  return SVNICP_ALIGN_SUCCESS;
}

static int fetch(svnicp_ctx* c, void* dst, const void* src, size_t bytes) {
  if (bind(c)) return SVNICP_ERR_HIP;
  HIPCHK(c, hipMemcpyAsync(dst, src, bytes, hipMemcpyDeviceToHost, c->stream));
  HIPCHK(c, hipStreamSynchronize(c->stream));
  return SVNICP_OK;
}
#define NEED_RESULT(c)                                                                   \
  do {                                                                                   \
    CTX_CHECK(c);                                                                        \
    if (!(c)->have_result) return fail((c), SVNICP_ERR_INVALID, "no registration result yet"); \
  } while (0)

static int fetch_stats(svnicp_ctx* c, void* dst, size_t off_doubles, size_t n_doubles) {
  if (c->host_stats_valid) { std::memcpy(dst, c->h_stats + off_doubles, n_doubles * 8); return SVNICP_OK; }
  return fetch(c, dst, c->stats.p + off_doubles, n_doubles * 8);
}
int svnicp_get_transformation(svnicp_ctx* c, double out6[6]) { NEED_RESULT(c); return fetch_stats(c, out6, 0, 6); }
int svnicp_get_distribution(svnicp_ctx* c, double out6[6]) { NEED_RESULT(c); return fetch_stats(c, out6, 6, 6); }
int svnicp_get_cov_matrix(svnicp_ctx* c, double out36[36]) { NEED_RESULT(c); return fetch_stats(c, out36, 12, 36); }
int svnicp_get_particle_weight(svnicp_ctx* c, double* outP) {
  NEED_RESULT(c);
  return fetch_stats(c, outP, 48, (size_t)c->P);
}
int svnicp_get_particles(svnicp_ctx* c, double* out6P) {
  CTX_CHECK(c);
  if (!c->particles_set) return fail(c, SVNICP_ERR_INVALID, "no particles set");
  return fetch(c, out6P, c->pose_out.p, (size_t)c->P * 48);
}
int svnicp_get_particle_history(svnicp_ctx* c, float* out) {
  NEED_RESULT(c);
  return fetch(c, out, c->history.p, (size_t)c->hist_I * 6 * c->hist_P * sizeof(float));
}

int svnicp_get_gpu_ms(svnicp_ctx* c, double out3[3]) {
  NEED_RESULT(c);
  if (bind(c)) return SVNICP_ERR_HIP;
  HIPCHK(c, hipStreamSynchronize(c->stream));
  float a = 0, b = 0;
  HIPCHK(c, hipEventElapsedTime(&a, c->ev[0], c->ev[1]));
  HIPCHK(c, hipEventElapsedTime(&b, c->ev[1], c->ev[2]));
  out3[0] = a; out3[1] = b; out3[2] = (double)a + b;
  return SVNICP_OK;
}

int svnicp_get_runtime(svnicp_ctx* c, double out3[3]) {
  NEED_RESULT(c);
  double ms[3];
  int rc = svnicp_get_gpu_ms(c, ms);
  if (rc) return rc;
  if (c->prm.mode == SVNICP_MODE_SVGD && c->prm.check_early_stop && !c->finish_seen) {
    int v[2] = {0, 0};
    HIPCHK(c, hipMemcpy(v, c->ctl.p, sizeof v, hipMemcpyDeviceToHost));
    if (v[0]) c->finish_iter = v[1];
    c->finish_seen = true;
  }
  out3[0] = ms[0] * 1e-3; out3[1] = ms[1] * 1e-3; out3[2] = (double)c->finish_iter;
  return SVNICP_OK;
}

int svnicp_get_iterations_run(svnicp_ctx* c, int* out) {
  NEED_RESULT(c);
  if (!out) return SVNICP_ERR_INVALID;
  int v[2];
  const int rc = fetch(c, v, c->ctl.p, sizeof v);
  if (rc) return rc;
  *out = v[1];
  return SVNICP_OK;
}

int svnicp_get_knn_fallbacks(svnicp_ctx* c, int* out) {
  CTX_CHECK(c);
  if (!c->have_candidates) return fail(c, SVNICP_ERR_INVALID, "no candidates yet");
  if (c->knn_variant == 0) { *out = -1; return SVNICP_OK; }
  return fetch(c, out, (c->tune.full_corr && c->stage_fail_count.p) ? c->stage_fail_count.p : c->fail_count.p, sizeof(int));
}

int svnicp_get_knn_fallback_rows(svnicp_ctx* c, int32_t* out, int cap, int* n_out) {
  CTX_CHECK(c);
  if (!c->have_candidates || !n_out) return fail(c, SVNICP_ERR_INVALID, "no candidates yet");
  *n_out = 0;
  if (c->knn_variant == 0) return SVNICP_OK;
  const bool snap = c->tune.full_corr && c->stage_fail_count.p;
  int n = 0;
  int rc = fetch(c, &n, snap ? c->stage_fail_count.p : c->fail_count.p, sizeof(int));
  if (rc) return rc;
  *n_out = n;
  if (n > cap) n = cap;
  if (n > 0 && out) return fetch(c, out, snap ? c->stage_fail_list.p : c->fail_list.p, (size_t)n * 4);
  return SVNICP_OK;
}

int svnicp_get_knn_survivors(svnicp_ctx* c, int32_t* outB) {
  CTX_CHECK(c);
  if (!c->have_candidates || c->knn_variant != 2 || !c->prm.record_trace || !c->stat_n.p)
    return fail(c, SVNICP_ERR_INVALID, "svnicp_get_knn_survivors: needs record_trace and the pruned stage-A kernel");
  return fetch(c, outB, c->stat_n.p, (size_t)c->B * 4);
}

int svnicp_get_ambiguous_steps(svnicp_ctx* c, int* out) {
  CTX_CHECK(c);
  if (!c->have_result) return fail(c, SVNICP_ERR_INVALID, "no registration result yet");
  if (c->accum_mode == 0) { *out = -1; return SVNICP_OK; }
  return fetch(c, out, c->ambig.p, sizeof(int));
}

int svnicp_get_ambiguous_pairs(svnicp_ctx* c, int64_t* out) {
  CTX_CHECK(c);
  if (!c->have_result || !out) return fail(c, SVNICP_ERR_INVALID, "no registration result yet");
  if (c->accum_mode != 3 || c->plan.f32 != 3) { *out = -1; return SVNICP_OK; }
  int v[2] = {0, 0};
  const int rc = fetch(c, v, c->ambig.p, sizeof v);
  *out = v[1];
  return rc;
}

int svnicp_set_profile(svnicp_ctx* c, int on) {
  CTX_CHECK(c);
  c->profile = on != 0;
  c->profile_mask = on == 1 ? ~0u : ((unsigned)on >> 1);
  return SVNICP_OK;
}

int svnicp_get_kernel_ms(svnicp_ctx* c, double* ms5, int32_t* launches5) {
  NEED_RESULT(c);
  if (!c->profile) return fail(c, SVNICP_ERR_INVALID, "svnicp_get_kernel_ms: profiling is off (svnicp_set_profile)");
  if (bind(c)) return SVNICP_ERR_HIP;
  HIPCHK(c, hipStreamSynchronize(c->stream));
  for (int i = 0; i < KC_COUNT; ++i) { ms5[i] = 0.0; launches5[i] = 0; }
  for (size_t i = 0; i < c->pused; ++i) {
    float ms = 0;
    HIPCHK(c, hipEventElapsedTime(&ms, c->pev[2 * i], c->pev[2 * i + 1]));
    ms5[c->pcls[i]] += ms;
    launches5[c->pcls[i]] += 1;
  }
  return SVNICP_OK;
}

int svnicp_get_candidates(svnicp_ctx* c, int32_t* out) {
  CTX_CHECK(c);
  if (!c->have_candidates) return fail(c, SVNICP_ERR_INVALID, "no candidates yet");
  return fetch(c, out, c->cand_idx.p, (size_t)c->B * c->K * 4);
}
int svnicp_get_candidate_dist2(svnicp_ctx* c, double* out) {
  CTX_CHECK(c);
  if (!c->have_candidates) return fail(c, SVNICP_ERR_INVALID, "no candidates yet");
  return fetch(c, out, c->cand_d2.p, (size_t)c->B * c->K * 8);
}

int svnicp_get_trace(svnicp_ctx* c, int32_t* corr, double* H, double* b, double* N, double* phi, double* h) {
  NEED_RESULT(c);
  if (!c->prm.record_trace) return fail(c, SVNICP_ERR_INVALID, "svnicp_get_trace: params.record_trace was 0");
  const size_t I = (size_t)c->prm.iterations, P = (size_t)c->P;
  int rc = 0;
  if (corr && (rc = fetch(c, corr, c->trcorr.p, I * P * (size_t)c->B * 4))) return rc;
  if (H && (rc = fetch(c, H, c->trH.p, I * P * 36 * 8))) return rc;
  if (b && (rc = fetch(c, b, c->trb.p, I * P * 6 * 8))) return rc;
  if (N && (rc = fetch(c, N, c->trN.p, I * P * 6 * 8))) return rc;
  if (phi && (rc = fetch(c, phi, c->trphi.p, I * P * 6 * 8))) return rc;
  if (h && (rc = fetch(c, h, c->trh.p, I * 8))) return rc;
  return SVNICP_OK;
}

}
```

svn-icp_amd/csrc/kernels.hpp:

```cpp
#pragma once
#include "device_math.hpp"

namespace svnicp {

struct KnnArgs {
  const double* src;
  Pose0 pose;
  const double *tx, *ty, *tz;
  const int32_t* torig;
  int64_t M, Mp;
  int64_t b_lo, b_hi;
  int K, S;
  double* pool_d;
  int32_t* pool_i;
  int32_t* out_idx;
  double* out_d2;
  const int32_t* qlist;
  const int* qlist_count;
  int list_grid;
  int list_qw;
  int slices, slice_max_queries, merge_n;
  double* sl_d;
  int32_t* sl_i;
  const double* qthr;
};
int knn_pool_size(int K);
int knn_slice_count(int K);
hipError_t launch_knn_merge_slices(const KnnArgs& a, hipStream_t st);
int64_t knn_padded_targets(int64_t M);

struct KnnBruteArgs {
  const double* src;
  Pose0 pose;
  const double* tgt;
  int64_t M;
  int64_t b_lo, b_hi;
  int K;
  int32_t* out_idx;
  double* out_d2;
  unsigned long long* phase_cycles;
};
bool knn_brute_applicable(int64_t B, int64_t M, int K);
int knn_brute_queries_per_block(int64_t n, int num_cus);
hipError_t launch_knn_brute(const KnnBruteArgs& a, int num_cus, int queries_per_block, hipStream_t st);

struct KnnScanArgs {
  const double* src;
  Pose0 pose;
  const double *tx, *ty, *tz;
  const float *txf, *tyf, *tzf;
  const int32_t* torig;
  const unsigned long long* emax_bits;
  int64_t M, Mp, Ms;
  int64_t b_lo, b_hi;
  int K, S2, seed_rank;
  int32_t* pool;
  int32_t* out_idx;
  double* out_d2;
  int32_t* fail_list;
  int* fail_count;
};
bool knn_scan_plan(int64_t Mp, int K, int64_t* Ms, int* seed_rank, int* S2);
hipError_t launch_targets_soa2(const double* tgt, int64_t M, int64_t Mp, double* tx, double* ty, double* tz,
                               float* txf, float* tyf, float* tzf, int32_t* torig, unsigned long long* emax_bits,
                               hipStream_t st);
hipError_t launch_knn_scan(const KnnScanArgs& a, hipStream_t st);
hipError_t launch_knn_topk(const KnnArgs& a, hipStream_t st);
hipError_t launch_build_table(const int32_t* idx, int64_t n_entries, const double* tgt, double* table,
                              hipStream_t st);

struct KnnTilesArgs {
  const double* src;
  Pose0 pose;
  const int32_t* qorder;
  const double *tx, *ty, *tz;
  const float *txf, *tyf, *tzf;
  const int32_t* torig;
  const float* tile_box;
  const unsigned long long* emax_bits;
  int64_t M, Mp;
  int n_tiles;
  int64_t b_lo, b_hi;
  int K, S2;
  int32_t* pool;
  int32_t* arena;
  int32_t* chunk_tab;
  int arena_cap;
  int64_t tab_rows;
  int scan_split;
  unsigned int group_stride;
  int32_t* out_idx;
  double* out_d2;
  int32_t* fail_list;
  int* fail_count;
  int32_t* stat_n;
  unsigned long long* phase_cycles;
  void* qrec;
  double* fail_tau;
};
constexpr int kTilesBase = 512, kTilesChunk = 512, kTilesChunks = 31;
bool knn_tiles_applicable(int64_t Mp, int K);
hipError_t launch_knn_tiles(const KnnTilesArgs& a, hipStream_t st);
size_t sort_temp_bytes(size_t n);
hipError_t launch_bbox(const double* pts, int64_t n, unsigned long long* bbox, hipStream_t st);
hipError_t launch_morton_order(const double* pts, int64_t i0, int64_t n, int transform, const Pose0& pose,
                               const unsigned long long* bbox, unsigned int* keys_a, unsigned int* keys_b,
                               int32_t* vals_a, int32_t* order, void* temp, size_t temp_bytes, hipStream_t st);
hipError_t launch_targets_sorted(const double* tgt, int64_t M, int64_t Mp, const int32_t* order, double* tx, double* ty,
                                 double* tz, float* txf, float* tyf, float* tzf, int32_t* torig, float* tile_box,
                                 unsigned long long* emax_bits, hipStream_t st);

struct AccumArgs {
  const double* src;
  const double* table;
  const float4* tablef;
  const float4* tablea;
  const float* cmax;
  int* ambig_count;
  const double* Rtot;
  int64_t B;
  int K, RS;
  int p_lo, p_hi;
  int TP;
  int tiles_per_block;
  int64_t n_tiles;
  int Ppad;
  double max_dist;
  double* partial;
  const int* ctl;
  int32_t* corr;
  int svgd;
  const double* tgt;
  const int32_t* cand;
  const double* anchor;
  int64_t M;
  uint8_t* kbest;
  int32_t* kidx;
  const int32_t* full_idx;
  int pts_per_block, spts_per_block;
  unsigned int* ticket;
  int fin_iteration, fin_P;
  double fin_thr;
  const double* fin_norms;
  const double* fin_pose;
  float* fin_history;
  int* fin_ctl;
};
struct AccumPlan { int PW, WP, TP, grid_x, grid_y, tiles_per_block, Ppad, RS, f32, K, sgrid_x, pts_per_block, spts_per_block; int64_t n_tiles; size_t smem;
                   int small;  };
constexpr int kSmallChainBlocks = 32;
struct Tuning {
  int knn = -1;
  int fallback_sliced_max = -1;
  int accum = 3;
  int update_fused = 0;
  int fused_update_max_p = 128;
  int wgpcu_search = 0, wgpcu_accum = 0;
  int tp = 0;
  int accum_min_steps = 0;
  int group_stride = 0;
  int scan_split = 0;
  int debug = 0;
  int single_fused = 1;
  int small_chain = 1;
  int persistent = 0;
  int median_inline = -1;
  int brute_qb = 0;
  int full_corr = 0;
};
AccumPlan plan_accumulate(int n_particles, int64_t B, int K, int num_cus, int f32, const Tuning& tune);
hipError_t launch_search_split(const AccumPlan& plan, AccumArgs a, hipStream_t st);
hipError_t launch_accumulate_split(const AccumPlan& plan, const AccumArgs& a, hipStream_t st);
void split_occupancy_blocks(int PW, int WP, int K, size_t smem, int* search, int* accum);
hipError_t launch_build_table3(const int32_t* idx, int64_t B, int K, const double* tgt, int64_t M, double* table,
                               double* anchor, float4* tablea, float* cmax, hipStream_t st);
hipError_t launch_build_table2(const int32_t* idx, int64_t B, int K, const double* tgt, int64_t M, double* table,
                               float4* tablef, float* cmax, hipStream_t st);
hipError_t launch_transform_cloud(const double* src, int64_t B, const double* pose12, double* q, const int* ctl, hipStream_t st);
struct UpdateArgs {
  const double* sums;
  int n_ranks;
  int sums_stride;
  double* sums_out;
  double* R;
  double* t;
  double* Rtot;
  Pose0 pose;
  int P, iteration, iterations;
  double lr, conv_thr;
  int check_early_stop, full_grad;
  double* work;
  float* history;
  double* pose_out;
  int* ctl;
  double *trH, *trb, *trN, *trphi, *trh;
  int h_in_lds;
  double* eul;
  double* opt;
  int svgd;
  int optimizer;
  double n_src;
  double* uctl;
  unsigned long long* dbg;
};
size_t update_workspace_doubles(int P);
struct BeginZero { unsigned int* ptr[6]; unsigned int dwords[6]; int n; int* ctl; int iterations; };
hipError_t launch_init_particles(const double* init6xP, int P, const Pose0& pose, int mode, double* R, double* t,
                                 double* Rtot, double* pose_out, int refresh_pose, double* eul, hipStream_t st, const BeginZero* zero = nullptr);
bool accumulate_can_fuse_single(const AccumPlan& plan);
int single_particle_grid(int64_t B);
hipError_t launch_accumulate(const AccumPlan& plan, AccumArgs a, const UpdateArgs* single, hipStream_t st);
hipError_t launch_update_svgd(const UpdateArgs& a, hipStream_t st);
hipError_t launch_update(const UpdateArgs& a, hipStream_t st);
hipError_t launch_update_median(const UpdateArgs& a, int num_cus, int max_p_one_workgroup, hipStream_t st);
hipError_t launch_update_prepare(const UpdateArgs& a, hipStream_t st);
hipError_t launch_update_prepare_median(const UpdateArgs& a, hipStream_t st);
bool small_registration_supported(int PW, int WP, int K);
hipError_t launch_small_registration(const AccumPlan& plan, AccumArgs a, const UpdateArgs& u, int iterations, unsigned int* bar,
                                     int num_cus, hipStream_t st);
hipError_t launch_update_direction(const UpdateArgs& a, hipStream_t st, bool finish = true);
const double* update_step_norms(const UpdateArgs& a);
hipError_t launch_reduce_partials(const double* partial, int nblk, int Ppad, int p_lo, int n_particles, double* sums, const int* ctl,
                                  hipStream_t st);
size_t update_uctl_doubles(int P);
struct StatsArgs { const double* pose; int P; int mode; double* out;  };
hipError_t launch_stats(const StatsArgs& a, hipStream_t st);

}
```

svn-icp_amd/csrc/spatial_prep.hip:

```cpp
#include <cstring>

#include <rocprim/device/device_radix_sort.hpp>

#include "kernels.hpp"

namespace svnicp {

namespace {

__device__ __forceinline__ unsigned long long enc_f64(double v) {
  const long long b = __double_as_longlong(v);
  return b < 0 ? ~(unsigned long long)b : ((unsigned long long)b | 0x8000000000000000ull);
}
__device__ __forceinline__ double dec_f64(unsigned long long e) {
  const unsigned long long b = (e & 0x8000000000000000ull) ? (e & 0x7fffffffffffffffull) : ~e;
  return __longlong_as_double((long long)b);
}
__device__ __forceinline__ float next_down(float f) {
  if (f == 0.0f) return -1.401298464e-45f;
  int b = __float_as_int(f);
  b += (f > 0.0f) ? -1 : 1;
  return __int_as_float(b);
}
__device__ __forceinline__ float next_up(float f) {
  if (f == 0.0f) return 1.401298464e-45f;
  int b = __float_as_int(f);
  b += (f > 0.0f) ? 1 : -1;
  return __int_as_float(b);
}
__device__ __forceinline__ float f32_floor(double v) { float f = (float)v; return ((double)f > v) ? next_down(f) : f; }
__device__ __forceinline__ float f32_ceil(double v) { float f = (float)v; return ((double)f < v) ? next_up(f) : f; }

__global__ __launch_bounds__(256) void k_bbox(const double* __restrict__ pts, int64_t n, unsigned long long* __restrict__ bbox) {
  double lo[3] = {__builtin_huge_val(), __builtin_huge_val(), __builtin_huge_val()};
  double hi[3] = {-__builtin_huge_val(), -__builtin_huge_val(), -__builtin_huge_val()};
  for (int64_t i = (int64_t)blockIdx.x * blockDim.x + threadIdx.x; i < n; i += (int64_t)gridDim.x * blockDim.x) {
#pragma unroll
    for (int d = 0; d < 3; ++d) { const double v = pts[3 * i + d]; lo[d] = fmin(lo[d], v); hi[d] = fmax(hi[d], v); }
  }
#pragma unroll
  for (int d = 0; d < 3; ++d) {
    for (int off = 32; off > 0; off >>= 1) {
      lo[d] = fmin(lo[d], __shfl_xor(lo[d], off, kWave));
      hi[d] = fmax(hi[d], __shfl_xor(hi[d], off, kWave));
    }
  }
  __shared__ double s_lo[4][3], s_hi[4][3];
  const int wave = threadIdx.x >> 6;
  if ((threadIdx.x & 63) == 0) {
#pragma unroll
    for (int d = 0; d < 3; ++d) { s_lo[wave][d] = lo[d]; s_hi[wave][d] = hi[d]; }
  }
  __syncthreads();
  if (threadIdx.x < 3) {
    const int d = threadIdx.x;
    double l = s_lo[0][d], h = s_hi[0][d];
    for (int w = 1; w < 4; ++w) { l = fmin(l, s_lo[w][d]); h = fmax(h, s_hi[w][d]); }
    if (l <= h) { atomicMin(&bbox[d], enc_f64(l)); atomicMax(&bbox[3 + d], enc_f64(h)); }
  }
}


__device__ __forceinline__ unsigned int spread10(unsigned int v) {
  v &= 0x3ffu;
  v = (v | (v << 16)) & 0x030000ffu;
  v = (v | (v << 8)) & 0x0300f00fu;
  v = (v | (v << 4)) & 0x030c30c3u;
  v = (v | (v << 2)) & 0x09249249u;
  return v;
}

__global__ void k_morton_keys(const double* __restrict__ pts, int64_t i0, int64_t n, int transform, Pose0 pose,
                              const unsigned long long* __restrict__ bbox, unsigned int* __restrict__ keys,
                              int32_t* __restrict__ vals) {
  const int64_t e = (int64_t)blockIdx.x * blockDim.x + threadIdx.x;
  if (e >= n) return;
  const int64_t i = i0 + e;
  double p[3] = {pts[3 * i], pts[3 * i + 1], pts[3 * i + 2]};
  if (transform) {
    const double* R = pose.R0;
    const double x = (p[0] * R[0] + p[1] * R[1] + p[2] * R[2]) + pose.t0[0];
    const double y = (p[0] * R[3] + p[1] * R[4] + p[2] * R[5]) + pose.t0[1];
    const double z = (p[0] * R[6] + p[1] * R[7] + p[2] * R[8]) + pose.t0[2];
    p[0] = x; p[1] = y; p[2] = z;
  }
  unsigned int c[3];
#pragma unroll
  for (int d = 0; d < 3; ++d) {
    const double lo = dec_f64(bbox[d]), hi = dec_f64(bbox[3 + d]);
    double u = (hi > lo) ? (p[d] - lo) / (hi - lo) : 0.0;
    if (!(u > 0.0)) u = 0.0;
    if (u > 0.999999) u = 0.999999;
    c[d] = (unsigned int)(u * 1024.0);
  }
  keys[e] = spread10(c[0]) | (spread10(c[1]) << 1) | (spread10(c[2]) << 2);
  vals[e] = (int32_t)i;
}

__global__ __launch_bounds__(256) void k_targets_sorted(const double* __restrict__ tgt, int64_t M,
                                                        const int32_t* __restrict__ order, double* __restrict__ tx,
                                                        double* __restrict__ ty, double* __restrict__ tz,
                                                        float* __restrict__ txf, float* __restrict__ tyf,
                                                        float* __restrict__ tzf, int32_t* __restrict__ torig,
                                                        float* __restrict__ tile_box , int n_tiles,
                                                        unsigned long long* __restrict__ emax_bits) {
  __shared__ float red[4][6];
  const int tile = blockIdx.x;
  float lo[3] = {__builtin_huge_valf(), __builtin_huge_valf(), __builtin_huge_valf()};
  float hi[3] = {-__builtin_huge_valf(), -__builtin_huge_valf(), -__builtin_huge_valf()};
  double e = 0.0;
  for (int r = threadIdx.x; r < 512; r += 256) {
    const int64_t j = (int64_t)tile * 512 + r;
    const double nan = __builtin_nan("");
    double x = nan, y = nan, z = nan;
    int32_t o = 0;
    if (j < M) {
      o = order[j];
      x = tgt[3 * (int64_t)o]; y = tgt[3 * (int64_t)o + 1]; z = tgt[3 * (int64_t)o + 2];
      const double m = fmax(fabs(x), fmax(fabs(y), fabs(z)));
      e = fmax(e, (m == m) ? m : __builtin_huge_val());
      if (x == x) { lo[0] = __builtin_fminf(lo[0], f32_floor(x)); hi[0] = __builtin_fmaxf(hi[0], f32_ceil(x)); }
      if (y == y) { lo[1] = __builtin_fminf(lo[1], f32_floor(y)); hi[1] = __builtin_fmaxf(hi[1], f32_ceil(y)); }
      if (z == z) { lo[2] = __builtin_fminf(lo[2], f32_floor(z)); hi[2] = __builtin_fmaxf(hi[2], f32_ceil(z)); }
    }
    tx[j] = x; ty[j] = y; tz[j] = z;
    txf[j] = (float)x; tyf[j] = (float)y; tzf[j] = (float)z;
    torig[j] = o;
  }
  for (int off = 32; off > 0; off >>= 1) {
#pragma unroll
    for (int d = 0; d < 3; ++d) {
      lo[d] = __builtin_fminf(lo[d], __shfl_xor(lo[d], off, kWave));
      hi[d] = __builtin_fmaxf(hi[d], __shfl_xor(hi[d], off, kWave));
    }
    e = fmax(e, __shfl_xor(e, off, kWave));
  }
  const int wave = threadIdx.x >> 6, lane = threadIdx.x & 63;
  if (lane == 0) {
#pragma unroll
    for (int d = 0; d < 3; ++d) { red[wave][d] = lo[d]; red[wave][3 + d] = hi[d]; }
    if (e > 0.0) atomicMax(emax_bits, (unsigned long long)__double_as_longlong(e));
  }
  __syncthreads();
  if (threadIdx.x < 6) {
    const int d = threadIdx.x;
    float v = red[0][d];
    for (int w = 1; w < 4; ++w) v = d < 3 ? __builtin_fminf(v, red[w][d]) : __builtin_fmaxf(v, red[w][d]);
    tile_box[(size_t)d * n_tiles + tile] = v;
  }
}

}

size_t sort_temp_bytes(size_t n) {
  size_t bytes = 0;
  (void)rocprim::radix_sort_pairs(nullptr, bytes, (unsigned int*)nullptr, (unsigned int*)nullptr, (int32_t*)nullptr,
                                  (int32_t*)nullptr, n, 0, 30, (hipStream_t)0);
  return bytes;
}

hipError_t launch_morton_order(const double* pts, int64_t i0, int64_t n, int transform, const Pose0& pose,
                               const unsigned long long* bbox, unsigned int* keys_a, unsigned int* keys_b,
                               int32_t* vals_a, int32_t* order, void* temp, size_t temp_bytes, hipStream_t st) {
  if (n <= 0) return hipSuccess;
  hipLaunchKernelGGL(k_morton_keys, dim3((unsigned)((n + 255) / 256)), dim3(256), 0, st, pts, i0, n, transform, pose, bbox,
                     keys_a, vals_a);
  hipError_t e = hipGetLastError();
  if (e != hipSuccess) return e;
  return rocprim::radix_sort_pairs(temp, temp_bytes, keys_a, keys_b, vals_a, order, (size_t)n, 0, 30, st);
}

hipError_t launch_bbox(const double* pts, int64_t n, unsigned long long* bbox, hipStream_t st) {
  hipError_t e = hipMemsetAsync(bbox, 0xff, 3 * sizeof(unsigned long long), st);
  if (e != hipSuccess) return e;
  e = hipMemsetAsync(bbox + 3, 0, 3 * sizeof(unsigned long long), st);
  if (e != hipSuccess) return e;
  int64_t nb = (n + 255) / 256;
  if (nb > 256) nb = 256;
  hipLaunchKernelGGL(k_bbox, dim3((unsigned)nb), dim3(256), 0, st, pts, n, bbox);
  return hipGetLastError();
}

hipError_t launch_targets_sorted(const double* tgt, int64_t M, int64_t Mp, const int32_t* order, double* tx, double* ty,
                                 double* tz, float* txf, float* tyf, float* tzf, int32_t* torig, float* tile_box,
                                 unsigned long long* emax_bits, hipStream_t st) {
  hipError_t e = hipMemsetAsync(emax_bits, 0, sizeof(unsigned long long), st);
  if (e != hipSuccess) return e;
  const int n_tiles = (int)(Mp / 512);
  hipLaunchKernelGGL(k_targets_sorted, dim3(n_tiles), dim3(256), 0, st, tgt, M, order, tx, ty, tz, txf, tyf, tzf, torig,
                     tile_box, n_tiles, emax_bits);
  return hipGetLastError();
}

}
```

svn-icp_amd/solver.py:

```python
from __future__ import annotations

import ctypes as C
import enum
from dataclasses import dataclass

import numpy as np

from . import binding
from .binding import Params, SvnIcpError

_OPT = {"Adam": 0, "RMSprop": 1, "SGD": 2, "Adagrad": 3}


class SteinICPState(enum.IntEnum):
    ALIGN_SUCCESS = 1
    NO_OPTIMIZER = 2


@dataclass
class SteinICPParam:
    iterations: int = 50
    use_minibatch: bool = False
    batch_size: int = 50
    lr: float = 0.02
    max_dist: float = 1.0
    normalize_cloud: bool = True
    optimizer: str = "Adam"
    check_early_stop: bool = False
    convergence_steps: int = 5
    convergence_threshold: float = 1e-5
    KNN_count: int = 100
    SVN_full_grad: bool = True
    record_trace: bool = False


@dataclass
class ParticleWeightOpt:
    use_weight_mean: bool = False


def initialize_particles(particle_count: int, ub, lb, rng: np.random.Generator | None = None) -> np.ndarray:
    if particle_count == 1:
        return np.zeros((6, 1))
    rng = rng or np.random.default_rng()
    ub, lb = np.asarray(ub, np.float64).reshape(6, 1), np.asarray(lb, np.float64).reshape(6, 1)
    return (ub - lb) * rng.random((6, particle_count)) + lb


def _is_torch_cuda(x) -> bool:
    return hasattr(x, "is_cuda") and bool(x.is_cuda)


class _SolverBase:
    _mode = 0

    def __init__(self, parameters: SteinICPParam, init_pose, opt: ParticleWeightOpt | None = None, device: int = 0):
        self._L = binding.load_library()
        self._h = C.c_void_p()
        self.config = parameters
        self.weight_config = opt or ParticleWeightOpt()
        init = self._pose_arg(init_pose)
        self._P = init.shape[1]
        prm = Params(C.sizeof(Params), self._mode, int(parameters.iterations), int(parameters.KNN_count),
                     float(parameters.lr), float(parameters.max_dist), float(parameters.convergence_threshold),
                     int(parameters.check_early_stop), int(parameters.SVN_full_grad),
                     _OPT.get(parameters.optimizer, -1), int(parameters.record_trace))
        rc = self._L.svnicp_create(C.byref(prm), int(device), init.ctypes.data_as(C.POINTER(C.c_double)), self._P,
                                   C.byref(self._h))
        if rc != 0:
            raise SvnIcpError(f"svnicp_create failed ({rc}): {self._L.svnicp_last_error(None).decode()}")
        self._B = self._M = 0
        self._K = int(parameters.KNN_count)
        self._keep = None

    @staticmethod
    def _pose_arg(init_pose) -> np.ndarray:
        if hasattr(init_pose, "detach"):
            init_pose = init_pose.detach().cpu().numpy()
        a = np.ascontiguousarray(np.asarray(init_pose, np.float64))
        if a.ndim == 3:
            a = a.reshape(a.shape[0], a.shape[1])
        if a.ndim != 2 or a.shape[0] != 6:
            raise ValueError("init_pose must be [6, P] (or [6, P, 1])")
        return np.ascontiguousarray(a)

    def _check(self, rc: int, what: str):
        if rc < 0:
            raise SvnIcpError(f"{what} failed ({rc}): {self._L.svnicp_last_error(self._h).decode()}")
        return rc

    def close(self):
        if getattr(self, "_h", None) and self._h.value:
            self._L.svnicp_destroy(self._h)
            self._h = C.c_void_p()

    def __del__(self):
        try:
            self.close()
        except Exception:
            pass

    @property
    def handle(self):
        return self._h

    def add_cloud(self, new_cloud, target, init_pose):
        if _is_torch_cuda(new_cloud) != _is_torch_cuda(target):
            raise ValueError("source and target must live on the same side (both host or both device)")
        if _is_torch_cuda(new_cloud):
            import torch
            src = new_cloud.to(torch.float64).contiguous()
            tgt = target.to(torch.float64).contiguous()
            torch.cuda.current_stream(src.device).synchronize()
            self._keep = (src, tgt)
            B, M = src.shape[0], tgt.shape[0]
            rc = self._L.svnicp_set_clouds(self._h, C.c_void_p(src.data_ptr()), B, C.c_void_p(tgt.data_ptr()), M, 1)
            self._check(rc, "svnicp_set_clouds")
        else:
            src = np.ascontiguousarray(np.asarray(new_cloud, np.float64).reshape(-1, 3))
            tgt = np.ascontiguousarray(np.asarray(target, np.float64).reshape(-1, 3))
            B, M = src.shape[0], tgt.shape[0]
            rc = self._L.svnicp_set_clouds(self._h, src.ctypes.data_as(C.c_void_p), B, tgt.ctypes.data_as(C.c_void_p),
                                           M, 0)
            self._check(rc, "svnicp_set_clouds")
        self._B, self._M = B, M
        init = self._pose_arg(init_pose)
        self._P = init.shape[1]
        self._check(self._L.svnicp_set_particles(self._h, init.ctypes.data_as(C.POINTER(C.c_double)), self._P),
                    "svnicp_set_particles")

    def add_cloud_device_target(self, new_cloud, target_devptr: int, M: int, init_pose):
        src = np.ascontiguousarray(np.asarray(new_cloud, np.float64).reshape(-1, 3))
        self._check(self._L.svnicp_set_source(self._h, src.ctypes.data_as(C.c_void_p), src.shape[0], 0), "svnicp_set_source")
        self._check(self._L.svnicp_set_target(self._h, C.c_void_p(int(target_devptr)), int(M), 1), "svnicp_set_target")
        self._B, self._M = src.shape[0], int(M)
        init = self._pose_arg(init_pose)
        self._P = init.shape[1]
        self._check(self._L.svnicp_set_particles(self._h, init.ctypes.data_as(C.POINTER(C.c_double)), self._P),
                    "svnicp_set_particles")

    def add_cloud_device(self, source_devptr: int, B: int, target_devptr: int, M: int, init_pose):
        self._check(self._L.svnicp_set_source(self._h, C.c_void_p(int(source_devptr)), int(B), 1), "svnicp_set_source")
        self._check(self._L.svnicp_set_target(self._h, C.c_void_p(int(target_devptr)), int(M), 1), "svnicp_set_target")
        self._B, self._M = int(B), int(M)
        init = self._pose_arg(init_pose)
        self._P = init.shape[1]
        self._check(self._L.svnicp_set_particles(self._h, init.ctypes.data_as(C.POINTER(C.c_double)), self._P),
                    "svnicp_set_particles")

    def set_initial_mean(self, pose):
        if isinstance(pose, (tuple, list)) and len(pose) == 2:
            R, t = np.asarray(pose[0], np.float64).reshape(3, 3), np.asarray(pose[1], np.float64).reshape(3)
        else:
            T = np.asarray(pose, np.float64).reshape(4, 4)
            R, t = T[:3, :3], T[:3, 3]
        R = np.ascontiguousarray(R).reshape(9)
        t = np.ascontiguousarray(t)
        dp = C.POINTER(C.c_double)
        self._check(self._L.svnicp_set_initial_mean(self._h, R.ctypes.data_as(dp), t.ctypes.data_as(dp)),
                    "svnicp_set_initial_mean")

    def set_k(self, k: int):
        self._K = int(k)
        self._check(self._L.svnicp_set_k(self._h, int(k)), "svnicp_set_k")

    def set_option(self, name: str, value) -> None:
        self._check(self._L.svnicp_set_option(self._h, str(name).encode(), str(value).encode()), "svnicp_set_option")

    def set_threshold(self, max_dist: float):
        self._check(self._L.svnicp_set_max_dist(self._h, float(max_dist)), "svnicp_set_max_dist")

    def stein_align(self) -> SteinICPState:
        return SteinICPState(self._check(self._L.svnicp_align(self._h), "svnicp_align"))

    def stein_align_async(self):
        self._check(self._L.svnicp_align_async(self._h), "svnicp_align_async")

    def synchronize(self):
        self._check(self._L.svnicp_synchronize(self._h), "svnicp_synchronize")

    def _getd(self, name: str, n: int) -> np.ndarray:
        out = np.zeros(n, np.float64)
        self._check(getattr(self._L, "svnicp_get_" + name)(self._h, out.ctypes.data_as(C.POINTER(C.c_double))),
                    "svnicp_get_" + name)
        return out

    def get_transformation(self) -> np.ndarray:
        return self._getd("transformation", 6)

    def get_distribution(self) -> np.ndarray:
        return self._getd("distribution", 6)

    def get_cov_matrix(self) -> np.ndarray:
        return self._getd("cov_matrix", 36)

    def get_particles(self) -> np.ndarray:
        return self._getd("particles", 6 * self._P)

    def get_particle_weight(self) -> np.ndarray:
        return self._getd("particle_weight", self._P)

    def get_particle_history(self) -> np.ndarray:
        out = np.zeros((int(self.config.iterations), 6 * self._P), np.float32)
        self._check(self._L.svnicp_get_particle_history(self._h, out.ctypes.data_as(C.POINTER(C.c_float))),
                    "svnicp_get_particle_history")
        return out

    def get_runtime(self) -> np.ndarray:
        return self._getd("runtime", 3)

    def get_gpu_ms(self) -> np.ndarray:
        return self._getd("gpu_ms", 3)

    KERNEL_CLASSES = ("stage_a_knn", "k_build_table", "k_stein_search", "k_stein_accumulate", "k_reduce_partials",
                      "k_particle_update")

    def set_profile(self, on, classes=None):
        v = int(bool(on))
        if on and classes:
            v = 0
            for k in classes:
                v |= 1 << (self.KERNEL_CLASSES.index(k) + 1)
        self._check(self._L.svnicp_set_profile(self._h, v), "svnicp_set_profile")

    def get_kernel_ms(self) -> dict:
        ms = np.zeros(len(self.KERNEL_CLASSES), np.float64)
        n = np.zeros(len(self.KERNEL_CLASSES), np.int32)
        self._check(self._L.svnicp_get_kernel_ms(self._h, ms.ctypes.data_as(C.POINTER(C.c_double)),
                                                 n.ctypes.data_as(C.POINTER(C.c_int32))), "svnicp_get_kernel_ms")
        return {k: (float(ms[i]), int(n[i])) for i, k in enumerate(self.KERNEL_CLASSES)}

    def get_candidates(self) -> np.ndarray:
        out = np.zeros((self._B, self._K), np.int32)
        self._check(self._L.svnicp_get_candidates(self._h, out.ctypes.data_as(C.POINTER(C.c_int32))),
                    "svnicp_get_candidates")
        return out

    def get_knn_fallbacks(self) -> int:
        v = C.c_int(0)
        self._check(self._L.svnicp_get_knn_fallbacks(self._h, C.byref(v)), "svnicp_get_knn_fallbacks")
        return int(v.value)

    def get_knn_fallback_rows(self) -> np.ndarray:
        n = C.c_int(0)
        out = np.zeros(max(1, self._B), np.int32)
        self._check(self._L.svnicp_get_knn_fallback_rows(self._h, out.ctypes.data_as(C.POINTER(C.c_int32)), out.size,
                                                         C.byref(n)), "svnicp_get_knn_fallback_rows")
        return out[:max(0, min(int(n.value), out.size))].copy()

    def get_knn_survivors(self) -> np.ndarray:
        out = np.zeros(self._B, np.int32)
        self._check(self._L.svnicp_get_knn_survivors(self._h, out.ctypes.data_as(C.POINTER(C.c_int32))),
                    "svnicp_get_knn_survivors")
        return out

    def get_iterations_run(self) -> int:
        v = C.c_int(0)
        self._check(self._L.svnicp_get_iterations_run(self._h, C.byref(v)), "svnicp_get_iterations_run")
        return int(v.value)

    def get_ambiguous_steps(self) -> int:
        v = C.c_int(0)
        self._check(self._L.svnicp_get_ambiguous_steps(self._h, C.byref(v)), "svnicp_get_ambiguous_steps")
        return int(v.value)

    def get_ambiguous_pairs(self) -> int:
        v = C.c_int64(0)
        self._check(self._L.svnicp_get_ambiguous_pairs(self._h, C.byref(v)), "svnicp_get_ambiguous_pairs")
        return int(v.value)

    def get_candidate_dist2(self) -> np.ndarray:
        return self._getd("candidate_dist2", self._B * self._K).reshape(self._B, self._K)

    def get_trace(self, with_corr: bool = True) -> dict:
        I, P, B = int(self.config.iterations), self._P, self._B
        d = dict(H=np.zeros((I, P, 36)), b=np.zeros((I, P, 6)), newton=np.zeros((I, P, 6)), phi=np.zeros((I, P, 6)),
                 h=np.zeros(I))
        corr = np.zeros((I, P, B), np.int32) if with_corr else None
        dp = C.POINTER(C.c_double)
        rc = self._L.svnicp_get_trace(self._h, corr.ctypes.data_as(C.POINTER(C.c_int32)) if with_corr else None,
                                      d["H"].ctypes.data_as(dp), d["b"].ctypes.data_as(dp),
                                      d["newton"].ctypes.data_as(dp), d["phi"].ctypes.data_as(dp),
                                      d["h"].ctypes.data_as(dp))
        self._check(rc, "svnicp_get_trace")
        if with_corr:
            d["corr"] = corr
        return d


class SVNICP(_SolverBase):
    _mode = 0


class SVGDICP(_SolverBase):
    _mode = 1
```

Before: 144.9 registrations/s.

## Replace rocprim radix sort with custom 3-pass Morton sort and fuse prologue memsets

Replaces the library radix sort used for Morton ordering of target and source points with a custom three-pass, 10-bit-digit LSD radix sort: histogram, scan and scatter kernels over 2048-item tiles, with the first histogram fused into the key-generation kernel. The bbox reduction now writes per-block partials that the key kernel combines, which removes the atomics and the memsets. Zeroing of emax and fail_count also moves into kernels. The goal is fewer launches and memsets in the per-alignment prologue, at the cost of a large hand-written sort that must match the library's ordering and stability, with the library kept as a fallback.

```diff
diff --git a/include/svnicp_hip.h b/include/svnicp_hip.h
--- a/include/svnicp_hip.h
+++ b/include/svnicp_hip.h
@@ -121,6 +121,8 @@
 int svnicp_get_knn_survivors(svnicp_ctx *ctx, int32_t *outB);
 int svnicp_get_ambiguous_steps(svnicp_ctx *ctx, int *out);
 int svnicp_get_ambiguous_pairs(svnicp_ctx *ctx, int64_t *out);
+int svnicp_get_prologue_launches(svnicp_ctx *ctx, int *counted, int *expected);
+int svnicp_debug_morton_order(svnicp_ctx *ctx, const double *pts, int64_t n, uint32_t *keys_out, int32_t *order_out);
 #define SVNICP_KERNEL_CLASSES 6
 int svnicp_set_profile(svnicp_ctx *ctx, int on);
 int svnicp_get_kernel_ms(svnicp_ctx *ctx, double *ms6, int32_t *launches6);
diff --git a/svn-icp_amd/binding.py b/svn-icp_amd/binding.py
--- a/svn-icp_amd/binding.py
+++ b/svn-icp_amd/binding.py
@@ -124,6 +124,8 @@
     L.svnicp_get_ambiguous_steps.argtypes = [vp, C.POINTER(C.c_int)]
     L.svnicp_get_ambiguous_pairs.argtypes = [vp, C.POINTER(C.c_int64)]
     L.svnicp_get_iterations_run.argtypes = [vp, C.POINTER(C.c_int)]
+    L.svnicp_get_prologue_launches.argtypes = [vp, C.POINTER(C.c_int), C.POINTER(C.c_int)]
+    L.svnicp_debug_morton_order.argtypes = [vp, vp, C.c_int64, vp, vp]
     L.svnicp_set_profile.argtypes = [vp, C.c_int]
     L.svnicp_get_kernel_ms.argtypes = [vp, dp, ip]
     L.svnicp_set_shard.argtypes = [vp, C.c_int, C.c_int]
diff --git a/svn-icp_amd/csrc/api.hip b/svn-icp_amd/csrc/api.hip
--- a/svn-icp_amd/csrc/api.hip
+++ b/svn-icp_amd/csrc/api.hip
@@ -92,6 +92,12 @@
   DevBuf<float> tile_box;
   DevBuf<unsigned char> sort_tmp;
   size_t sort_tmp_bytes = 0;
+  DevBuf<int32_t> vals_b;
+  DevBuf<unsigned int> sort_hist, sort_ghist;
+  DevBuf<double> bbox_part;
+  int bbox_nparts = 0;
+  int prologue_enq = 0;
+  bool prologue_open = false;
   bool use_scan = false;
   int64_t scan_Ms = 0; int scan_rank = 0, scan_S2 = 0;
   DevBuf<float> history;
@@ -255,6 +261,7 @@
   for (auto* b : dbl) b->release();
   c->eul.release(); c->opt.release(); c->uctl.release(); c->rank_sums.release(); c->stage_fail_count.release(); c->stage_fail_list.release(); c->small_bar.release();
   c->keys_a.release(); c->keys_b.release(); c->vals_a.release(); c->order_t.release(); c->qorder.release(); c->stat_n.release(); c->bbox.release(); c->tile_box.release(); c->sort_tmp.release();
+  c->vals_b.release(); c->sort_hist.release(); c->sort_ghist.release(); c->bbox_part.release();
   c->full_q.release(); c->full_d2.release(); c->full_idx.release(); c->arena.release(); c->chunk_tab.release();
   c->pool_i.release(); c->torig.release(); c->pool2.release(); c->fail_list.release(); c->txf.release(); c->tyf.release(); c->tzf.release(); c->cmaxb.release(); c->tablef.release(); c->tablea.release(); c->kbest.release(); c->kidx.release(); c->sl_d.release(); c->sl_i.release(); c->fail_tau.release(); c->qrec.release(); c->anchor.release(); c->ambig.release(); c->emax.release(); c->fail_count.release(); c->cand_idx.release(); c->trcorr.release(); c->history.release(); c->ctl.release();
   if (c->dbg_phase) (void)hipFree(c->dbg_phase);
@@ -414,6 +421,7 @@
   else if (k == "chain") { if (v == "auto") { t.small_chain = 1; t.persistent = 0; } else if (v == "persistent") { t.small_chain = 1; t.persistent = 1; }
                            else if (v == "general") { t.small_chain = 0; t.persistent = 0; } else ok = false; }
   else if (k == "median") { if (v == "auto") t.median_inline = -1; else if (v == "stream") t.median_inline = 0; else if (v == "inline") t.median_inline = 1; else ok = false; }
+  else if (k == "sort") { if (v == "radix3") t.sort_library = 0; else if (v == "library") t.sort_library = 1; else ok = false; }
   else if (k == "correspondence") { if (v == "fast") t.full_corr = 0; else if (v == "full") t.full_corr = 1; else ok = false; }
   else return fail(c, SVNICP_ERR_INVALID, "svnicp_set_option: unknown option '" + k + "'");
   if (!ok) return fail(c, SVNICP_ERR_INVALID, "svnicp_set_option: bad value '" + v + "' for option '" + k + "'");
@@ -445,6 +453,29 @@
 }
 
 void* svnicp_rank_sums_devptr(svnicp_ctx* c) { return (c && c->row_world > 1) ? (void*)c->rank_sums.p : nullptr; }
+
+static size_t chunk_tab_words(int64_t B) { return (((size_t)B * kTilesChunks + 16 + (size_t)(B + 63) / 64 + 1) + 255) & ~(size_t)255; }
+
+static int ensure_sort_buffers(svnicp_ctx* c, size_t nmax) {
+  HIPCHK(c, c->vals_b.ensure(nmax));
+  HIPCHK(c, c->bbox_part.ensure((size_t)6 * kBboxParts));
+  HIPCHK(c, c->sort_hist.ensure(sort_hist_words(std::min<size_t>(nmax, (size_t)kSortMaxItems))));
+  if (!c->sort_ghist.p) {
+    HIPCHK(c, c->sort_ghist.ensure((size_t)3 * kSortBins));
+    HIPCHK(c, hipMemsetAsync(c->sort_ghist.p, 0, (size_t)3 * kSortBins * sizeof(unsigned int), c->stream));
+  }
+  if (c->tune.sort_library || nmax > (size_t)kSortMaxItems) {
+    const size_t tb = sort_temp_bytes(nmax);
+    if (tb > c->sort_tmp_bytes) { HIPCHK(c, c->sort_tmp.ensure(tb)); c->sort_tmp_bytes = tb; }
+  }
+  return 0;
+}
+static MortonSortBuffers sort_buffers(const svnicp_ctx* c) {
+  MortonSortBuffers s{};
+  s.keys_a = c->keys_a.p; s.keys_b = c->keys_b.p; s.vals_a = c->vals_a.p; s.vals_b = c->vals_b.p;
+  s.hist = c->sort_hist.p; s.ghist = c->sort_ghist.p; s.temp = c->sort_tmp.p; s.temp_bytes = c->sort_tmp_bytes;
+  return s;
+}
 
 static int ensure_target_layout(svnicp_ctx* c) {
   int want = 0;
@@ -472,11 +503,12 @@
     HIPCHK(c, c->order_t.ensure((size_t)M)); HIPCHK(c, c->qorder.ensure((size_t)c->B));
     HIPCHK(c, c->bbox.ensure(6));
     HIPCHK(c, c->tile_box.ensure((size_t)6 * (Mp / 512)));
-    const size_t tb = sort_temp_bytes(nmax);
-    if (tb > c->sort_tmp_bytes) { HIPCHK(c, c->sort_tmp.ensure(tb)); c->sort_tmp_bytes = tb; }
-    HIPCHK(c, launch_bbox(c->tgt.p, M, c->bbox.p, c->stream));
-    HIPCHK(c, launch_morton_order(c->tgt.p, 0, M, 0, c->pose0, c->bbox.p, c->keys_a.p, c->keys_b.p, c->vals_a.p,
-                                  c->order_t.p, c->sort_tmp.p, c->sort_tmp_bytes, c->stream));
+    if (const int rc = ensure_sort_buffers(c, nmax)) return rc;
+    HIPCHK(c, launch_bbox(c->tgt.p, M, c->bbox_part.p, &c->bbox_nparts, c->emax.p, c->stream));
+    c->prologue_enq += 1;
+    HIPCHK(c, launch_morton_order(c->tgt.p, 0, M, 0, c->pose0, c->bbox.p, c->bbox_part.p, c->bbox_nparts, sort_buffers(c),
+                                  c->order_t.p, c->tune.sort_library != 0, nullptr, &c->prologue_enq, c->stream));
+    c->prologue_enq += 1;
     HIPCHK(c, launch_targets_sorted(c->tgt.p, M, Mp, c->order_t.p, c->tx.p, c->ty.p, c->tz.p, c->txf.p, c->tyf.p, c->tzf.p,
                                     c->torig.p, c->tile_box.p, c->emax.p, c->stream));
   }
@@ -493,6 +525,7 @@
   const int64_t B = c->B;
   c->S = knn_pool_size(c->K);
   HIPCHK(c, hipEventRecord(c->ev[0], c->stream));
+  c->prologue_enq = 0; c->prologue_open = true;
   if (ensure_target_layout(c)) return c->err.empty() ? SVNICP_ERR_HIP : SVNICP_ERR_HIP;
   if (c->knn_variant == 3) {
     HIPCHK(c, c->fail_count.ensure(1));
@@ -502,7 +535,7 @@
       c->arena_cap = (int)std::max<int64_t>(32768, B / 4);
       HIPCHK(c, c->pool2.ensure((size_t)B * kTilesBase));
       HIPCHK(c, c->arena.ensure((size_t)c->arena_cap * kTilesChunk));
-      HIPCHK(c, c->chunk_tab.ensure((size_t)B * kTilesChunks + 16 + (size_t)(B + 63) / 64 + 1));
+      HIPCHK(c, c->chunk_tab.ensure(chunk_tab_words(B)));
     } else {
       HIPCHK(c, c->pool2.ensure((size_t)B * c->scan_S2));
     }
@@ -564,6 +597,7 @@
     HIPCHK(c, hipMemsetAsync(c->trN.p, 0, (size_t)I * P * 6 * 8, c->stream));
     HIPCHK(c, hipMemsetAsync(c->trphi.p, 0, (size_t)I * P * 6 * 8, c->stream));
     HIPCHK(c, hipMemsetAsync(c->trh.p, 0, ((size_t)I + 1) * 8, c->stream));
+    c->prologue_enq += 6;
   }
   c->pused = 0;
   c->single_done_it = -1;
@@ -589,6 +623,7 @@
     z.ctl = c->ctl.p; z.iterations = I;
     HIPCHK(c, launch_init_particles(c->init_pose.p, P, c->pose0, 2, c->R.p, c->t.p, c->Rtot.p, c->pose_out.p, 0,
                                     nullptr, c->stream, &z));
+    c->prologue_enq += 1;
   }
   c->particles_dirty = false;
   c->began = true;
@@ -639,8 +674,9 @@
   } else if (c->knn_variant == 2) {
     const int64_t n = b_hi - b_lo;
     if (n > 0) {
-      HIPCHK(c, launch_morton_order(qsrc, b_lo, n, 1, pose, c->bbox.p, c->keys_a.p, c->keys_b.p, c->vals_a.p,
-                                    c->qorder.p + b_lo, c->sort_tmp.p, c->sort_tmp_bytes, c->stream));
+      int enq = 0;
+      HIPCHK(c, launch_morton_order(qsrc, b_lo, n, 1, pose, c->bbox.p, nullptr, 0, sort_buffers(c), c->qorder.p + b_lo,
+                                    c->tune.sort_library != 0, c->fail_count.p, &enq, c->stream));
       KnnTilesArgs k{};
       k.src = qsrc; k.pose = pose; k.qorder = c->qorder.p + b_lo;
       k.tx = c->tx.p; k.ty = c->ty.p; k.tz = c->tz.p; k.txf = c->txf.p; k.tyf = c->tyf.p; k.tzf = c->tzf.p;
@@ -657,11 +693,11 @@
         if (ng <= 2 || st >= ng) st = 1;
         k.group_stride = st;
       }
-      HIPCHK(c, hipMemsetAsync(c->chunk_tab.p, 0xff, ((size_t)c->B * kTilesChunks + 16 + (size_t)(c->B + 63) / 64 + 1) * sizeof(int32_t), c->stream));
+      HIPCHK(c, hipMemsetAsync(c->chunk_tab.p, 0xff, chunk_tab_words(c->B) * sizeof(int32_t), c->stream));
+      if (c->prologue_open) { c->prologue_enq += enq + 1; c->prologue_open = false; }
       k.fail_list = c->fail_list.p; k.fail_count = c->fail_count.p; k.fail_tau = c->fail_tau.p; k.qrec = c->qrec.p;
       a.qthr = c->fail_tau.p;
       if (c->prm.record_trace) { HIPCHK(c, c->stat_n.ensure((size_t)c->B)); k.stat_n = c->stat_n.p; }
-      HIPCHK(c, hipMemsetAsync(c->fail_count.p, 0, sizeof(int), c->stream));
       unsigned long long*& dbg_phase = c->dbg_phase;
       const size_t dbg_waves = (size_t)((n + 63) / 64) * 4;
       if (c->tune.debug && dbg_waves <= 65536) {
@@ -1117,6 +1153,37 @@
   return SVNICP_OK;
 }
 
+int svnicp_get_prologue_launches(svnicp_ctx* c, int* counted, int* expected) {
+  CTX_CHECK(c);
+  if (!c->have_candidates || !counted || !expected) return fail(c, SVNICP_ERR_INVALID, "no candidates yet");
+  *counted = c->prologue_enq;
+  *expected = c->knn_variant == 2 ? kPrologueLaunchesTiles : -1;
+  return SVNICP_OK;
+}
+
+int svnicp_debug_morton_order(svnicp_ctx* c, const double* pts, int64_t n, uint32_t* keys_out, int32_t* order_out) {
+  CTX_CHECK(c);
+  if (!pts || n < 1 || n > 0x7fffffffLL || !keys_out || !order_out) return fail(c, SVNICP_ERR_INVALID, "svnicp_debug_morton_order: bad argument");
+  if (bind(c)) return SVNICP_ERR_HIP;
+  DevBuf<double> d_pts; DevBuf<int32_t> d_order;
+  struct Free { DevBuf<double>& a; DevBuf<int32_t>& b; ~Free() { a.release(); b.release(); } } fr{d_pts, d_order};
+  HIPCHK(c, d_pts.ensure((size_t)n * 3)); HIPCHK(c, d_order.ensure((size_t)n));
+  HIPCHK(c, c->keys_a.ensure((size_t)n)); HIPCHK(c, c->keys_b.ensure((size_t)n)); HIPCHK(c, c->vals_a.ensure((size_t)n));
+  HIPCHK(c, c->bbox.ensure(6)); HIPCHK(c, c->emax.ensure(1));
+  if (const int rc = ensure_sort_buffers(c, (size_t)n)) return rc;
+  c->target_layout = -1;
+  HIPCHK(c, hipMemcpyAsync(d_pts.p, pts, (size_t)n * 24, hipMemcpyHostToDevice, c->stream));
+  HIPCHK(c, launch_bbox(d_pts.p, n, c->bbox_part.p, &c->bbox_nparts, c->emax.p, c->stream));
+  HIPCHK(c, launch_morton_order(d_pts.p, 0, n, 0, c->pose0, c->bbox.p, c->bbox_part.p, c->bbox_nparts, sort_buffers(c), d_order.p,
+                                c->tune.sort_library != 0, nullptr, nullptr, c->stream));
+  MortonSortBuffers kb = sort_buffers(c);
+  HIPCHK(c, hipMemcpyAsync(order_out, d_order.p, (size_t)n * 4, hipMemcpyDeviceToHost, c->stream));
+  HIPCHK(c, launch_morton_keys_only(d_pts.p, n, c->pose0, c->bbox.p, kb.keys_b, kb.vals_b, c->stream));
+  HIPCHK(c, hipMemcpyAsync(keys_out, kb.keys_b, (size_t)n * 4, hipMemcpyDeviceToHost, c->stream));
+  HIPCHK(c, hipStreamSynchronize(c->stream));
+  return SVNICP_OK;
+}
+
 int svnicp_get_candidates(svnicp_ctx* c, int32_t* out) {
   CTX_CHECK(c);
   if (!c->have_candidates) return fail(c, SVNICP_ERR_INVALID, "no candidates yet");
diff --git a/svn-icp_amd/csrc/kernels.hpp b/svn-icp_amd/csrc/kernels.hpp
--- a/svn-icp_amd/csrc/kernels.hpp
+++ b/svn-icp_amd/csrc/kernels.hpp
@@ -101,11 +101,27 @@
 constexpr int kTilesBase = 512, kTilesChunk = 512, kTilesChunks = 31;
 bool knn_tiles_applicable(int64_t Mp, int K);
 hipError_t launch_knn_tiles(const KnnTilesArgs& a, hipStream_t st);
+constexpr int kSortTile = 2048, kSortBins = 1024, kSortMaxTiles = 1024;
+constexpr int64_t kSortMaxItems = (int64_t)kSortTile * kSortMaxTiles;
+constexpr int kBboxParts = 256;
+constexpr int kMortonOrderLaunches = 9;
+constexpr int kLibrarySortLaunches = 11;
+constexpr int kPrologueLaunchesTiles = 1 + kMortonOrderLaunches + 1 + 1 + kMortonOrderLaunches + 1;
+struct MortonSortBuffers {
+  unsigned int *keys_a, *keys_b;
+  int32_t *vals_a, *vals_b;
+  unsigned int* hist;
+  unsigned int* ghist;
+  void* temp; size_t temp_bytes;
+};
 size_t sort_temp_bytes(size_t n);
-hipError_t launch_bbox(const double* pts, int64_t n, unsigned long long* bbox, hipStream_t st);
+size_t sort_hist_words(size_t n);
+hipError_t launch_bbox(const double* pts, int64_t n, double* part, int* n_part, unsigned long long* zero64, hipStream_t st);
 hipError_t launch_morton_order(const double* pts, int64_t i0, int64_t n, int transform, const Pose0& pose,
-                               const unsigned long long* bbox, unsigned int* keys_a, unsigned int* keys_b,
-                               int32_t* vals_a, int32_t* order, void* temp, size_t temp_bytes, hipStream_t st);
+                               unsigned long long* bbox, const double* part, int n_part, const MortonSortBuffers& s,
+                               int32_t* order, bool library, int* zero32, int* launches, hipStream_t st);
+hipError_t launch_morton_keys_only(const double* pts, int64_t n, const Pose0& pose, unsigned long long* bbox, unsigned int* keys,
+                                   int32_t* vals, hipStream_t st);
 hipError_t launch_targets_sorted(const double* tgt, int64_t M, int64_t Mp, const int32_t* order, double* tx, double* ty,
                                  double* tz, float* txf, float* tyf, float* tzf, int32_t* torig, float* tile_box,
                                  unsigned long long* emax_bits, hipStream_t st);
@@ -166,6 +182,7 @@
   int persistent = 0;
   int median_inline = -1;
   int brute_qb = 0;
+  int sort_library = 0;
   int full_corr = 0;
 };
 AccumPlan plan_accumulate(int n_particles, int64_t B, int K, int num_cus, int f32, const Tuning& tune);
diff --git a/svn-icp_amd/csrc/spatial_prep.hip b/svn-icp_amd/csrc/spatial_prep.hip
--- a/svn-icp_amd/csrc/spatial_prep.hip
+++ b/svn-icp_amd/csrc/spatial_prep.hip
@@ -31,7 +31,9 @@
 __device__ __forceinline__ float f32_floor(double v) { float f = (float)v; return ((double)f > v) ? next_down(f) : f; }
 __device__ __forceinline__ float f32_ceil(double v) { float f = (float)v; return ((double)f < v) ? next_up(f) : f; }
 
-__global__ __launch_bounds__(256) void k_bbox(const double* __restrict__ pts, int64_t n, unsigned long long* __restrict__ bbox) {
+__global__ __launch_bounds__(256) void k_bbox(const double* __restrict__ pts, int64_t n, double* __restrict__ part,
+                                              unsigned long long* __restrict__ zero64) {
+  if (zero64 && blockIdx.x == 0 && threadIdx.x == 0) *zero64 = 0ull;
   double lo[3] = {__builtin_huge_val(), __builtin_huge_val(), __builtin_huge_val()};
   double hi[3] = {-__builtin_huge_val(), -__builtin_huge_val(), -__builtin_huge_val()};
   for (int64_t i = (int64_t)blockIdx.x * blockDim.x + threadIdx.x; i < n; i += (int64_t)gridDim.x * blockDim.x) {
@@ -56,7 +58,7 @@
     const int d = threadIdx.x;
     double l = s_lo[0][d], h = s_hi[0][d];
     for (int w = 1; w < 4; ++w) { l = fmin(l, s_lo[w][d]); h = fmax(h, s_hi[w][d]); }
-    if (l <= h) { atomicMin(&bbox[d], enc_f64(l)); atomicMax(&bbox[3 + d], enc_f64(h)); }
+    part[6 * blockIdx.x + d] = l; part[6 * blockIdx.x + 3 + d] = h;
   }
 }
 
@@ -70,31 +72,194 @@
   return v;
 }
 
-__global__ void k_morton_keys(const double* __restrict__ pts, int64_t i0, int64_t n, int transform, Pose0 pose,
-                              const unsigned long long* __restrict__ bbox, unsigned int* __restrict__ keys,
-                              int32_t* __restrict__ vals) {
-  const int64_t e = (int64_t)blockIdx.x * blockDim.x + threadIdx.x;
-  if (e >= n) return;
-  const int64_t i = i0 + e;
-  double p[3] = {pts[3 * i], pts[3 * i + 1], pts[3 * i + 2]};
-  if (transform) {
-    const double* R = pose.R0;
-    const double x = (p[0] * R[0] + p[1] * R[1] + p[2] * R[2]) + pose.t0[0];
-    const double y = (p[0] * R[3] + p[1] * R[4] + p[2] * R[5]) + pose.t0[1];
-    const double z = (p[0] * R[6] + p[1] * R[7] + p[2] * R[8]) + pose.t0[2];
-    p[0] = x; p[1] = y; p[2] = z;
-  }
-  unsigned int c[3];
-#pragma unroll
-  for (int d = 0; d < 3; ++d) {
-    const double lo = dec_f64(bbox[d]), hi = dec_f64(bbox[3 + d]);
-    double u = (hi > lo) ? (p[d] - lo) / (hi - lo) : 0.0;
-    if (!(u > 0.0)) u = 0.0;
-    if (u > 0.999999) u = 0.999999;
-    c[d] = (unsigned int)(u * 1024.0);
-  }
-  keys[e] = spread10(c[0]) | (spread10(c[1]) << 1) | (spread10(c[2]) << 2);
-  vals[e] = (int32_t)i;
+constexpr int kSortItems = kSortTile / 256;
+
+__device__ __forceinline__ unsigned int wave_sum(unsigned int v) {
+  for (int off = 32; off > 0; off >>= 1) v += __shfl_xor(v, off, kWave);
+  return v;
+}
+
+__global__ __launch_bounds__(256) void k_morton_keys(const double* __restrict__ pts, int64_t i0, int64_t n, int transform, Pose0 pose,
+                                                     unsigned long long* __restrict__ bbox, const double* __restrict__ part, int n_part,
+                                                     unsigned int* __restrict__ keys, int32_t* __restrict__ vals,
+                                                     unsigned int* __restrict__ hist0, unsigned int* __restrict__ ghist,
+                                                     int* __restrict__ zero32) {
+  __shared__ double s_box[4][6];
+  __shared__ unsigned int s_hist[kSortBins];
+  const int t = threadIdx.x, wave = t >> 6;
+  if (zero32 && blockIdx.x == 0 && t == 0) *zero32 = 0;
+  if (hist0)
+    for (int e = t; e < kSortBins; e += 256) s_hist[e] = 0u;
+  double blo[3], bhi[3];
+  if (part) {
+    double l[3] = {__builtin_huge_val(), __builtin_huge_val(), __builtin_huge_val()};
+    double h[3] = {-__builtin_huge_val(), -__builtin_huge_val(), -__builtin_huge_val()};
+    if (t < n_part) {
+#pragma unroll
+      for (int d = 0; d < 3; ++d) { l[d] = part[6 * t + d]; h[d] = part[6 * t + 3 + d]; }
+    }
+#pragma unroll
+    for (int d = 0; d < 3; ++d)
+      for (int off = 32; off > 0; off >>= 1) {
+        l[d] = fmin(l[d], __shfl_xor(l[d], off, kWave));
+        h[d] = fmax(h[d], __shfl_xor(h[d], off, kWave));
+      }
+    if ((t & 63) == 0) {
+#pragma unroll
+      for (int d = 0; d < 3; ++d) { s_box[wave][d] = l[d]; s_box[wave][3 + d] = h[d]; }
+    }
+    __syncthreads();
+#pragma unroll
+    for (int d = 0; d < 3; ++d) {
+      blo[d] = fmin(fmin(s_box[0][d], s_box[1][d]), fmin(s_box[2][d], s_box[3][d]));
+      bhi[d] = fmax(fmax(s_box[0][3 + d], s_box[1][3 + d]), fmax(s_box[2][3 + d], s_box[3][3 + d]));
+    }
+    if (blockIdx.x == 0 && t < 3) { bbox[t] = enc_f64(blo[t]); bbox[3 + t] = enc_f64(bhi[t]); }
+  } else {
+#pragma unroll
+    for (int d = 0; d < 3; ++d) { blo[d] = dec_f64(bbox[d]); bhi[d] = dec_f64(bbox[3 + d]); }
+    __syncthreads();
+  }
+  const int64_t tile0 = (int64_t)blockIdx.x * kSortTile;
+#pragma unroll 2
+  for (int j = 0; j < kSortItems; ++j) {
+    const int64_t e = tile0 + j * 256 + t;
+    if (e >= n) break;
+    const int64_t i = i0 + e;
+    double p[3] = {pts[3 * i], pts[3 * i + 1], pts[3 * i + 2]};
+    if (transform) {
+      const double* R = pose.R0;
+      const double x = (p[0] * R[0] + p[1] * R[1] + p[2] * R[2]) + pose.t0[0];
+      const double y = (p[0] * R[3] + p[1] * R[4] + p[2] * R[5]) + pose.t0[1];
+      const double z = (p[0] * R[6] + p[1] * R[7] + p[2] * R[8]) + pose.t0[2];
+      p[0] = x; p[1] = y; p[2] = z;
+    }
+    unsigned int c[3];
+#pragma unroll
+    for (int d = 0; d < 3; ++d) {
+      const double lo = blo[d], hi = bhi[d];
+      double u = (hi > lo) ? (p[d] - lo) / (hi - lo) : 0.0;
+      if (!(u > 0.0)) u = 0.0;
+      if (u > 0.999999) u = 0.999999;
+      c[d] = (unsigned int)(u * 1024.0);
+    }
+    const unsigned int key = spread10(c[0]) | (spread10(c[1]) << 1) | (spread10(c[2]) << 2);
+    keys[e] = key;
+    vals[e] = (int32_t)i;
+    if (hist0) atomicAdd(&s_hist[key & 1023u], 1u);
+  }
+  if (!hist0) return;
+  __syncthreads();
+  for (int bin = t; bin < kSortBins; bin += 256) {
+    const unsigned int v = s_hist[bin];
+    hist0[(size_t)blockIdx.x * kSortBins + bin] = v;
+    if (v) atomicAdd(&ghist[bin], v);
+  }
+}
+
+__global__ __launch_bounds__(256) void k_sort_hist(const unsigned int* __restrict__ keys, int64_t n, int shift, unsigned int* __restrict__ hist,
+                                                   unsigned int* __restrict__ ghist) {
+  __shared__ unsigned int sh[kSortBins];
+  const int t = threadIdx.x;
+  for (int e = t; e < kSortBins; e += 256) sh[e] = 0u;
+  __syncthreads();
+  const int64_t tile0 = (int64_t)blockIdx.x * kSortTile;
+#pragma unroll
+  for (int j = 0; j < kSortItems; ++j) {
+    const int64_t e = tile0 + j * 256 + t;
+    if (e < n) atomicAdd(&sh[(keys[e] >> shift) & 1023u], 1u);
+  }
+  __syncthreads();
+  for (int bin = t; bin < kSortBins; bin += 256) {
+    const unsigned int v = sh[bin];
+    hist[(size_t)blockIdx.x * kSortBins + bin] = v;
+    if (v) atomicAdd(&ghist[bin], v);
+  }
+}
+
+__global__ __launch_bounds__(256) void k_sort_scan(unsigned int* __restrict__ hist, int tiles, const unsigned int* __restrict__ ghist) {
+  const int lane = threadIdx.x & 63;
+  const int d = blockIdx.x * 4 + (threadIdx.x >> 6);
+  constexpr int kChunks = kSortMaxTiles / 64;
+  unsigned int v[kChunks];
+#pragma unroll
+  for (int c = 0; c < kChunks; ++c) {
+    const int tl = c * 64 + lane;
+    v[c] = tl < tiles ? hist[(size_t)tl * kSortBins + d] : 0u;
+  }
+  unsigned int base = 0u;
+  for (int i = lane; i < d; i += 64) base += ghist[i];
+  unsigned int carry = wave_sum(base);
+#pragma unroll
+  for (int c = 0; c < kChunks; ++c) {
+    if (c * 64 >= tiles) break;
+    unsigned int incl = v[c];
+    for (int off = 1; off < 64; off <<= 1) {
+      const unsigned int o = __shfl_up(incl, off, kWave);
+      if (lane >= off) incl += o;
+    }
+    const int tl = c * 64 + lane;
+    if (tl < tiles) hist[(size_t)tl * kSortBins + d] = carry + (incl - v[c]);
+    carry += __shfl(incl, 63, kWave);
+  }
+}
+
+template <bool LAST>
+__global__ __launch_bounds__(256) void k_sort_scatter(const unsigned int* __restrict__ keys_in, const int32_t* __restrict__ vals_in,
+                                                      unsigned int* __restrict__ keys_out, int32_t* __restrict__ vals_out, int64_t n,
+                                                      int shift, const unsigned int* __restrict__ offs,
+                                                      unsigned int* __restrict__ ghist_clear) {
+  __shared__ unsigned int wh[4][kSortBins];
+  const int t = threadIdx.x, w = t >> 6, lane = t & 63;
+  for (int e = t; e < 4 * kSortBins; e += 256) (&wh[0][0])[e] = 0u;
+  if (LAST && blockIdx.x == 0)
+    for (int e = t; e < 3 * kSortBins; e += 256) ghist_clear[e] = 0u;
+  const int64_t base = (int64_t)blockIdx.x * kSortTile + w * (kSortTile / 4);
+  unsigned int key[kSortItems], rank[kSortItems];
+  int32_t val[kSortItems];
+#pragma unroll
+  for (int j = 0; j < kSortItems; ++j) {
+    const int64_t e = base + j * 64 + lane;
+    key[j] = e < n ? keys_in[e] : 0u;
+    val[j] = e < n ? vals_in[e] : 0;
+  }
+  __syncthreads();
+  const unsigned long long below_mask = (1ull << lane) - 1ull;
+#pragma unroll
+  for (int j = 0; j < kSortItems; ++j) {
+    const bool valid = base + j * 64 + lane < n;
+    const unsigned int d = (key[j] >> shift) & 1023u;
+    unsigned long long same = __ballot(valid);
+#pragma unroll
+    for (int b = 0; b < 10; ++b) {
+      const bool bit = (d >> b) & 1u;
+      const unsigned long long m = __ballot(bit);
+      same &= bit ? m : ~m;
+    }
+    const unsigned int below = (unsigned int)__popcll(same & below_mask);
+    unsigned int pre = 0u;
+    if (valid) pre = wh[w][d];
+    __builtin_amdgcn_wave_barrier();
+    if (valid && below == 0u) wh[w][d] = pre + (unsigned int)__popcll(same);
+    __builtin_amdgcn_wave_barrier();
+    rank[j] = pre + below;
+  }
+  __syncthreads();
+  for (int bin = t; bin < kSortBins; bin += 256) {
+    const unsigned int c0 = wh[0][bin], c1 = wh[1][bin], c2 = wh[2][bin];
+    const unsigned int o = offs[(size_t)blockIdx.x * kSortBins + bin];
+    wh[0][bin] = o; wh[1][bin] = o + c0; wh[2][bin] = o + c0 + c1; wh[3][bin] = o + c0 + c1 + c2;
+  }
+  __syncthreads();
+#pragma unroll
+  for (int j = 0; j < kSortItems; ++j) {
+    if (base + j * 64 + lane >= n) continue;
+    const unsigned int d = (key[j] >> shift) & 1023u;
+    const unsigned int dest = wh[w][d] + rank[j];
+    if ((int64_t)dest >= n) continue;
+    vals_out[dest] = val[j];
+    if (!LAST) keys_out[dest] = key[j];
+  }
 }
 
 __global__ __launch_bounds__(256) void k_targets_sorted(const double* __restrict__ tgt, int64_t M,
@@ -152,40 +317,67 @@
 
 }
 
+using LibSortConfig = rocprim::radix_sort_config<rocprim::default_config, rocprim::default_config, rocprim::default_config, 0>;
+
 size_t sort_temp_bytes(size_t n) {
   size_t bytes = 0;
-  (void)rocprim::radix_sort_pairs(nullptr, bytes, (unsigned int*)nullptr, (unsigned int*)nullptr, (int32_t*)nullptr,
-                                  (int32_t*)nullptr, n, 0, 30, (hipStream_t)0);
+  (void)rocprim::radix_sort_pairs<LibSortConfig>(nullptr, bytes, (unsigned int*)nullptr, (unsigned int*)nullptr, (int32_t*)nullptr,
+                                                 (int32_t*)nullptr, n, 0, 30, (hipStream_t)0);
   return bytes;
 }
 
+size_t sort_hist_words(size_t n) { return ((n + kSortTile - 1) / kSortTile) * (size_t)kSortBins; }
+
 hipError_t launch_morton_order(const double* pts, int64_t i0, int64_t n, int transform, const Pose0& pose,
-                               const unsigned long long* bbox, unsigned int* keys_a, unsigned int* keys_b,
-                               int32_t* vals_a, int32_t* order, void* temp, size_t temp_bytes, hipStream_t st) {
+                               unsigned long long* bbox, const double* part, int n_part, const MortonSortBuffers& s,
+                               int32_t* order, bool library, int* zero32, int* launches, hipStream_t st) {
   if (n <= 0) return hipSuccess;
-  hipLaunchKernelGGL(k_morton_keys, dim3((unsigned)((n + 255) / 256)), dim3(256), 0, st, pts, i0, n, transform, pose, bbox,
-                     keys_a, vals_a);
-  hipError_t e = hipGetLastError();
-  if (e != hipSuccess) return e;
-  return rocprim::radix_sort_pairs(temp, temp_bytes, keys_a, keys_b, vals_a, order, (size_t)n, 0, 30, st);
-}
-
-hipError_t launch_bbox(const double* pts, int64_t n, unsigned long long* bbox, hipStream_t st) {
-  hipError_t e = hipMemsetAsync(bbox, 0xff, 3 * sizeof(unsigned long long), st);
-  if (e != hipSuccess) return e;
-  e = hipMemsetAsync(bbox + 3, 0, 3 * sizeof(unsigned long long), st);
-  if (e != hipSuccess) return e;
+  const int tiles = (int)((n + kSortTile - 1) / kSortTile);
+  if (library || n > kSortMaxItems) {
+    hipLaunchKernelGGL(k_morton_keys, dim3(tiles), dim3(256), 0, st, pts, i0, n, transform, pose, bbox, part, n_part, s.keys_a, s.vals_a,
+                       (unsigned int*)nullptr, (unsigned int*)nullptr, zero32);
+    hipError_t e = hipGetLastError();
+    if (e != hipSuccess) return e;
+    if (launches) *launches += 1 + kLibrarySortLaunches;
+    size_t temp_bytes = s.temp_bytes;
+    return rocprim::radix_sort_pairs<LibSortConfig>(s.temp, temp_bytes, s.keys_a, s.keys_b, s.vals_a, order, (size_t)n, 0, 30, st);
+  }
+  unsigned int* hist = s.hist;
+  hipLaunchKernelGGL(k_morton_keys, dim3(tiles), dim3(256), 0, st, pts, i0, n, transform, pose, bbox, part, n_part, s.keys_a, s.vals_a,
+                     hist, s.ghist, zero32);
+  hipLaunchKernelGGL(k_sort_scan, dim3(kSortBins / 4), dim3(256), 0, st, hist, tiles, s.ghist);
+  hipLaunchKernelGGL(k_sort_scatter<false>, dim3(tiles), dim3(256), 0, st, s.keys_a, s.vals_a, s.keys_b, s.vals_b, n, 0, hist,
+                     (unsigned int*)nullptr);
+  hipLaunchKernelGGL(k_sort_hist, dim3(tiles), dim3(256), 0, st, s.keys_b, n, 10, hist, s.ghist + kSortBins);
+  hipLaunchKernelGGL(k_sort_scan, dim3(kSortBins / 4), dim3(256), 0, st, hist, tiles, s.ghist + kSortBins);
+  hipLaunchKernelGGL(k_sort_scatter<false>, dim3(tiles), dim3(256), 0, st, s.keys_b, s.vals_b, s.keys_a, s.vals_a, n, 10, hist,
+                     (unsigned int*)nullptr);
+  hipLaunchKernelGGL(k_sort_hist, dim3(tiles), dim3(256), 0, st, s.keys_a, n, 20, hist, s.ghist + 2 * kSortBins);
+  hipLaunchKernelGGL(k_sort_scan, dim3(kSortBins / 4), dim3(256), 0, st, hist, tiles, s.ghist + 2 * kSortBins);
+  hipLaunchKernelGGL(k_sort_scatter<true>, dim3(tiles), dim3(256), 0, st, s.keys_a, s.vals_a, (unsigned int*)nullptr, order, n, 20, hist,
+                     s.ghist);
+  if (launches) *launches += kMortonOrderLaunches;
+  return hipGetLastError();
+}
+
+hipError_t launch_morton_keys_only(const double* pts, int64_t n, const Pose0& pose, unsigned long long* bbox, unsigned int* keys,
+                                   int32_t* vals, hipStream_t st) {
+  hipLaunchKernelGGL(k_morton_keys, dim3((unsigned)((n + kSortTile - 1) / kSortTile)), dim3(256), 0, st, pts, (int64_t)0, n, 0, pose, bbox,
+                     (const double*)nullptr, 0, keys, vals, (unsigned int*)nullptr, (unsigned int*)nullptr, (int*)nullptr);
+  return hipGetLastError();
+}
+
+hipError_t launch_bbox(const double* pts, int64_t n, double* part, int* n_part, unsigned long long* zero64, hipStream_t st) {
   int64_t nb = (n + 255) / 256;
-  if (nb > 256) nb = 256;
-  hipLaunchKernelGGL(k_bbox, dim3((unsigned)nb), dim3(256), 0, st, pts, n, bbox);
+  if (nb > kBboxParts) nb = kBboxParts;
+  *n_part = (int)nb;
+  hipLaunchKernelGGL(k_bbox, dim3((unsigned)nb), dim3(256), 0, st, pts, n, part, zero64);
   return hipGetLastError();
 }
 
 hipError_t launch_targets_sorted(const double* tgt, int64_t M, int64_t Mp, const int32_t* order, double* tx, double* ty,
                                  double* tz, float* txf, float* tyf, float* tzf, int32_t* torig, float* tile_box,
                                  unsigned long long* emax_bits, hipStream_t st) {
-  hipError_t e = hipMemsetAsync(emax_bits, 0, sizeof(unsigned long long), st);
-  if (e != hipSuccess) return e;
   const int n_tiles = (int)(Mp / 512);
   hipLaunchKernelGGL(k_targets_sorted, dim3(n_tiles), dim3(256), 0, st, tgt, M, order, tx, ty, tz, txf, tyf, tzf, torig,
                      tile_box, n_tiles, emax_bits);
diff --git a/svn-icp_amd/solver.py b/svn-icp_amd/solver.py
--- a/svn-icp_amd/solver.py
+++ b/svn-icp_amd/solver.py
@@ -236,6 +236,19 @@
                     "svnicp_get_candidates")
         return out
 
+    def get_prologue_launches(self):
+        a, b = C.c_int(0), C.c_int(0)
+        self._check(self._L.svnicp_get_prologue_launches(self._h, C.byref(a), C.byref(b)), "svnicp_get_prologue_launches")
+        return int(a.value), int(b.value)
+
+    def debug_morton_order(self, pts: np.ndarray):
+        pts = np.ascontiguousarray(pts, np.float64).reshape(-1, 3)
+        keys = np.zeros(pts.shape[0], np.uint32)
+        order = np.zeros(pts.shape[0], np.int32)
+        self._check(self._L.svnicp_debug_morton_order(self._h, pts.ctypes.data, pts.shape[0], keys.ctypes.data, order.ctypes.data),
+                    "svnicp_debug_morton_order")
+        return keys, order
+
     def get_knn_fallbacks(self) -> int:
         v = C.c_int(0)
         self._check(self._L.svnicp_get_knn_fallbacks(self._h, C.byref(v)), "svnicp_get_knn_fallbacks")
```

Result: no change. 146.3 registrations/s (median of 6 runs) (+0.9%).
